# Terascale-All-sensing-Research-Studio/MOV-SLAM

Hardware: AMD Instinct MI355X
Metric: local-BA iterations/sec (50 KF x 20k MapPoint window) (higher is better)
Workload: dtype f64; 1 GPU; LocalBundleAdjustment 50 KF + 10 fixed x 20000 MapPoints, E=110510 mono edges, Huber on, 10 LM iterations (cfg3, seed 1003); one window per GPU; parallelism=1 window

## Files before the change

mov-slam_amd/csrc/kernels.h:

```cpp
#pragma once
#include <hip/hip_runtime.h>

#include "device_types.h"

namespace movba {

constexpr int kBandThreads = 512;
constexpr int kPcgRowsThreads = 512;
constexpr int kPcgPlanWaves = kPcgRowsThreads / 64, kPcgPlanOwnBatch = 10;

hipError_t configure_kernels(int unused);
hipError_t configure_pcg_rows();
hipError_t configure_struct_kernels();
hipError_t launch_struct_count(const StructDev &sd, hipStream_t s);
hipError_t launch_struct_scan(const StructDev &sd, hipStream_t s);
hipError_t launch_struct_counts_out(const StructDev &sd, int32_t *host_cnt_dev, int seq, hipStream_t s, const int32_t *basic_pe = nullptr, const int32_t *basic_info = nullptr);
hipError_t launch_ingest(const IngestArgs &a, hipStream_t s);
int ingest_workgroups();
hipError_t launch_basic(const BasicDev &bd, hipStream_t s);
bool struct_lds_fits(int nfree, int NP);
hipError_t launch_struct_fill(const StructDev &sd, hipStream_t s);
hipError_t launch_couple_count(const StructDev &sd, int32_t *cnt_pt, hipStream_t s);
size_t sorted_fill_temp_bytes(int P, long long noff, int nfree);
hipError_t launch_sorted_fill(const StructDev &sd, const int32_t *cnt_pt, int32_t *off, unsigned *keys_in, unsigned *keys_out,
                              unsigned long long *vals_in, void *tmp, size_t tmp_bytes, long long noff, hipStream_t s);
hipError_t launch_slot_point(int32_t *slot, const int32_t *g_pose, const int32_t *base, const int32_t *g_point, int32_t *slot_point, int E, const int32_t *hx, int NP, hipStream_t s);
bool pcg_rows_supported(int nfree, const int32_t *row_ptr, PcgParams *pp);
hipError_t launch_pcg_rows(const DevWindow &w, int nrowent, const PcgParams &pp, int trial, hipStream_t s);

hipError_t launch_init(const DevWindow &w, hipStream_t s);
hipError_t launch_linearize(const DevWindow &w, hipStream_t s);
hipError_t launch_schur(const DevWindow &w, int mode, hipStream_t s);
hipError_t launch_lambda_init(const DevWindow &w, hipStream_t s);
hipError_t launch_backsub(const DevWindow &w, hipStream_t s);
hipError_t launch_finalize(const DevWindow &w, hipStream_t s);
struct ExportDst { unsigned long long *poses, *points, *chi2, *outlier; };
hipError_t launch_export(const DevWindow &w, const ExportDst &d, hipStream_t s);

hipError_t launch_init_batch(const BatchDev &b, int nblk, hipStream_t s);
hipError_t launch_point_batch(const BatchDev &b, int nblk, bool backsub, bool stereo, bool ldsp, size_t lds, hipStream_t s);
size_t point_lds_bytes_for(const DevWindow &w, bool backsub, bool ldsp);
int schur_blocks(const DevWindow &w);
hipError_t launch_schur_batch(const BatchDev &b, int nblk, int mode, bool stereo, hipStream_t s);
hipError_t launch_lambda_init_batch(const BatchDev &b, hipStream_t s);
hipError_t launch_finalize_batch(const BatchDev &b, int nblk, hipStream_t s);
hipError_t launch_pcg_rows_batch(const BatchDev &b, bool overflow, bool padded, size_t lds, int trial, hipStream_t s);
size_t pcg_rows_lds_bytes(int nfree, int nrowent, bool padded);
size_t band_lds_bytes(int nfree, int bw);
bool band_supported(int nfree, int bw);
hipError_t launch_band(const DevWindow &w, int bw, hipStream_t s);
hipError_t launch_band_batch(const BatchDev &b, size_t lds, hipStream_t s);
hipError_t configure_band();

hipError_t configure_dense_kernels();
hipError_t launch_dense_solve(const DevWindow &w, hipStream_t s);
hipError_t launch_dense_factor(const DevWindow &w, hipStream_t s);
hipError_t configure_dense_persist();
bool dense_persist_supported(const DensePlan &p);
hipError_t launch_dense_persist(const DevWindow &w, unsigned epoch, hipStream_t s);
size_t dense_tiles_doubles(int nfree);
int dense_ntile(int nfree);
constexpr size_t kPointLdsLimit = 150 * 1024;
size_t point_lds_need(int NP, int nfree);

}
```

mov-slam_amd/csrc/pcg_plan.cpp:

```cpp
#include "kernels.h"

namespace movba {

namespace {
constexpr int kNW = kPcgPlanWaves, kNC = kCoarseDim, kOwnBatch = kPcgPlanOwnBatch;
}

size_t pcg_rows_lds_bytes(int nfree, int nrowent, bool padded)
{
    const size_t n = 6 * (size_t)nfree, npad = (n + 1) & ~(size_t)1;
    const size_t ypart = padded ? n * kOwnBatch + 5 * kOwnBatch + 6 + kOwnBatch : 6 * ((size_t)nrowent / 2 + 1 + kOwnBatch);
    const size_t solve = (2 * npad + 36 * (size_t)nfree + 2 * kNW + 2 + kNC * kNC / 2 + kNC + 32 * kNW + ypart + 36 * (size_t)nfree + 64 * kNW) * sizeof(double);
    const size_t coarse = ((size_t)kNC * kNC + 9 * kNC + 8) * sizeof(double) + 2 * sizeof(int32_t) * ((size_t)nrowent + 2);
    return solve > coarse ? solve : coarse;
}

size_t band_lds_bytes(int nfree, int bw)
{
    const size_t n = 6 * (size_t)nfree, npad = (n + 1) & ~(size_t)1;
    const size_t ntri = ((size_t)bw * (bw + 1) / 2 + 1) & ~(size_t)1;
    return ((size_t)nfree * (bw + 1) * 36 + 2 * npad + (size_t)bw * 36 + 8 + 12) * sizeof(double) + (ntri + 4) * sizeof(int32_t);
}

bool band_supported(int nfree, int bw) { return nfree >= 1 && bw >= 0 && bw <= 77 && band_lds_bytes(nfree, bw) <= 159 * 1024; }

bool pcg_rows_supported(int nfree, const int32_t *row_ptr, PcgParams *pp)
{
    if (nfree <= 0 || nfree > 10 * kNW) return false;
    const int nrowent = row_ptr[nfree];
    int maxrow = 0;
    for (int b = 0; b < nfree; ++b) maxrow = row_ptr[b + 1] - row_ptr[b] > maxrow ? row_ptr[b + 1] - row_ptr[b] : maxrow;
    pp->padded = 0;
    if (pcg_rows_lds_bytes(nfree, nrowent, false) > 159 * 1024) return false;
    const bool pad_fits = maxrow <= 2 * kOwnBatch && pcg_rows_lds_bytes(nfree, nrowent, true) <= 159 * 1024;
    auto fill = [&](int cap, int32_t *out) {
        int b = 0, wv = 0;
        for (; wv < kNW && b < nfree; ++wv) {
            int e = b + 1;
            while (e < nfree && e - b < 10 && row_ptr[e + 1] - row_ptr[b] <= cap) ++e;
            if (out) out[wv + 1] = e;
            b = e;
        }
        if (out) for (; wv < kNW; ++wv) out[wv + 1] = nfree;
        return b == nfree;
    };
    if (nfree <= kNW) {
        for (int wv = 0; wv <= kNW; ++wv) pp->wave_row0[wv] = wv < nfree ? wv : nfree;
        pp->overflow = 0;
        pp->padded = pad_fits ? 1 : 0;
        return true;
    }
    int lo = 1, hi = nrowent > 1 ? nrowent : 1;
    while (lo < hi) {
        const int mid = (lo + hi) / 2;
        if (fill(mid, nullptr)) hi = mid; else lo = mid + 1;
    }
    pp->wave_row0[0] = 0;
    if (!fill(lo, pp->wave_row0)) return false;
    pp->overflow = 0;
    for (int wv = 0; wv < kNW; ++wv)
        if (row_ptr[pp->wave_row0[wv + 1]] - row_ptr[pp->wave_row0[wv]] > 128) pp->overflow = 1;
    pp->padded = (pad_fits && !pp->overflow) ? 1 : 0;
    return true;
}

}
```

mov-slam_amd/csrc/structure.cpp:

```cpp
#include "structure.h"

#include <algorithm>
#include <cstdlib>
#include <cstring>

namespace movba {

void reset_structure(Structure& s, int NP, int P, int E)
{
    s.nfree = 0; s.npairs = 0; s.nitems = 0; s.max_degree = 0; s.nentries = 0; s.already_grouped = true; s.n_fixed = 0; s.n_agg = 0; s.reordered = false;
    s.free_pose.clear(); s.pair_i.clear(); s.pair_j.clear(); s.items.clear(); s.sched.clear(); s.sched_per_xcd = 0; s.row_ent.clear();
    s.cblk_g.clear(); s.cblk_h.clear(); s.cblk_ptr.clear(); s.cblk_ent.clear(); s.ent_i.clear(); s.ent_j.clear(); s.ent_l.clear(); s.E_free = 0;
    s.NP = NP; s.P = P; s.E = E;
}

void index_poses(const uint8_t* pose_fixed, Structure& s)
{
    const int NP = s.NP;
    s.hidx.assign(NP, -1);
    std::vector<int32_t>& pstart = s.pose_slot0;
    pstart.assign(NP + 1, -1);
    int run = 0;
    for (int i = 0; i < NP; ++i) {
        if (pose_fixed[i]) { s.n_fixed++; continue; }
        if (s.pose_edges[i] > 0) { s.hidx[i] = s.nfree++; s.free_pose.push_back(i); pstart[i] = run; run += s.pose_edges[i]; }
    }
    s.E_free = run;
}

int build_basic(const movba_lba_desc& d, Structure& s, int32_t* rank_out)
{
    const int NP = d.n_poses, P = d.n_points, E = d.n_edges;
    if (NP < 0 || P < 0 || E < 0) return MOVBA_ERR_ARG;
    if ((NP && (!d.poses || !d.pose_fixed)) || (P && !d.points)) return MOVBA_ERR_ARG;
    if (E && (!d.edge_pose || !d.edge_point || !d.obs || !d.inv_sigma2)) return MOVBA_ERR_ARG;
    reset_structure(s, NP, P, E);

    s.pose_edges.assign(NP + 1, 0);
    s.pt_start.assign(P + 2, 0);
    {
        bool grouped = true;
        int prev_l = -1;
        int32_t *pe = s.pose_edges.data(), *pend = s.pt_start.data() + 1;
        const int32_t *ep = d.edge_pose, *el = d.edge_point;
        for (int e = 0; e < E; ++e) {
            const int ip = ep[e], l = el[e];
            if ((unsigned)ip >= (unsigned)NP || (unsigned)l >= (unsigned)P) return MOVBA_ERR_ARG;
            const int r = pe[ip]++;
            if (rank_out) rank_out[e] = r;
            pend[l] = e + 1;
            grouped &= l >= prev_l;
            prev_l = l;
        }
        s.already_grouped = grouped;
    }
    if (s.already_grouped) {
        for (int l = 0; l < P; ++l) {
            const int b = s.pt_start[l], en = std::max(s.pt_start[l + 1], b);
            s.pt_start[l + 1] = en;
            s.max_degree = std::max(s.max_degree, en - b);
        }
        s.pt_start.pop_back();
    } else {
        std::fill(s.pt_start.begin(), s.pt_start.end(), 0);
        for (int e = 0; e < E; ++e) s.pt_start[d.edge_point[e] + 2]++;
        for (int l = 0; l < P; ++l) { s.max_degree = std::max(s.max_degree, s.pt_start[l + 2]); s.pt_start[l + 2] += s.pt_start[l + 1]; }
    }
    if (s.already_grouped) {
        s.perm.clear();
        s.gp = d.edge_pose; s.gl = d.edge_point;
    } else {
        s.perm.resize(E);
        s.g_pose.resize(E); s.g_point.resize(E);
        for (int e = 0; e < E; ++e) {
            const int pos = s.pt_start[d.edge_point[e] + 1]++;
            s.perm[pos] = e;
        }
        s.pt_start.pop_back();
        for (int g = 0; g < E; ++g) {
            s.g_pose[g] = d.edge_pose[s.perm[g]];
            s.g_point[g] = d.edge_point[s.perm[g]];
        }
        s.gp = s.g_pose.data(); s.gl = s.g_point.data();
    }
    index_poses(d.pose_fixed, s);
    if (!rank_out) build_slots(s);
    if (E == 0) return MOVBA_EMPTY;
    return MOVBA_OK;
}

void build_slots(Structure& s)
{
    s.slot.resize(s.E);
    const int32_t *gp = s.gp;
    int32_t *sl = s.slot.data(), *ps = s.pose_slot0.data();
    for (int g = 0; g < s.E; ++g) { const int i = gp[g]; const int v = ps[i]; sl[g] = v; ps[i] = v + (v >= 0); }
}

static int free_lists(const Structure& s, std::vector<int32_t>& fe_start, std::vector<int32_t>& fe_h, std::vector<int32_t>& fe_g)
{
    const int P = s.P;
    fe_start.assign(P + 1, 0); fe_h.clear(); fe_g.clear();
    fe_h.reserve(s.E); fe_g.reserve(s.E);
    for (int l = 0; l < P; ++l) {
        const size_t base = fe_h.size();
        for (int g = s.pt_start[l]; g < s.pt_start[l + 1]; ++g) {
            const int h = s.hidx[s.gp[g]];
            if (h < 0) continue;
            size_t pos = fe_h.size();
            fe_h.push_back(h); fe_g.push_back(g);
            while (pos > base && fe_h[pos - 1] > h) {
                fe_h[pos] = fe_h[pos - 1]; fe_g[pos] = fe_g[pos - 1];
                --pos;
            }
            fe_h[pos] = h; fe_g[pos] = g;
            if (pos > base && fe_h[pos - 1] == h) return MOVBA_ERR_ARG;
            if (pos + 1 < fe_h.size() && fe_h[pos + 1] == h) return MOVBA_ERR_ARG;
        }
        fe_start[l + 1] = (int32_t)fe_h.size();
    }
    return MOVBA_OK;
}

int finish_pairs(Structure& s, const int32_t* cnt)
{
    const int nf = s.nfree;
    s.pid.assign((size_t)nf * (size_t)nf, -1);
    s.pair_i.clear(); s.pair_j.clear();
    for (int i = 0; i < nf; ++i) { s.pid[(size_t)i * nf + i] = i; s.pair_i.push_back(i); s.pair_j.push_back(i); }
    for (int i = 0; i < nf; ++i)
        for (int j = i + 1; j < nf; ++j)
            if (cnt[(size_t)i * nf + j] > 0) {
                s.pid[(size_t)i * nf + j] = (int32_t)s.pair_i.size();
                s.pair_i.push_back(i); s.pair_j.push_back(j);
            }
    s.npairs = (int)s.pair_i.size();
    s.pair_ptr.assign(s.npairs + 1, 0);
    for (int p = 0; p < s.npairs; ++p) s.pair_ptr[p + 1] = s.pair_ptr[p] + cnt[(size_t)s.pair_i[p] * nf + s.pair_j[p]];
    s.nentries = s.pair_ptr[s.npairs];
    if (s.nentries > (int64_t)0x7fffffff) return MOVBA_ERR_ARG;
    if (nf > 0 && s.pair_ptr[nf] != (int64_t)s.E_free) return MOVBA_ERR_ARG;

    s.items.clear();
    s.pair_item_start.assign(s.npairs + 1, 0);
    for (int p = 0; p < s.npairs; ++p) {
        const int64_t cap = p < nf ? kSchurChunkDiag : kSchurChunk, len = s.pair_ptr[p + 1] - s.pair_ptr[p];
        const int64_t parts = (len + cap - 1) / cap;
        const int64_t chunk = parts > 0 ? ((len + parts - 1) / parts + 3) / 4 * 4 : cap;
        s.pair_item_start[p] = (int32_t)s.items.size();
        for (int64_t b = s.pair_ptr[p]; b < s.pair_ptr[p + 1]; b += chunk)
            s.items.push_back(Item{ p, (int32_t)b, (int32_t)std::min<int64_t>(b + chunk, s.pair_ptr[p + 1]), p < nf ? 1 : 0 });
    }
    s.pair_item_start[s.npairs] = (int32_t)s.items.size();
    s.nitems = (int)s.items.size();

    {
        const int ipw = kSchurWaves / kSchurWPI;
        std::vector<int32_t>& order = s.tmp_order;
        order.resize(s.nitems);
        {
            int n = 0, od = nf < s.npairs ? s.pair_item_start[nf] : s.nitems;
            for (int i = 0; i < nf; ++i) {
                for (int k = s.pair_item_start[i]; k < s.pair_item_start[i + 1]; ++k) order[n++] = k;
                while (od < s.nitems && s.pair_i[s.items[od].pair] == i) order[n++] = od++;
            }
        }
        auto weight = [&](int k) { const Item& it = s.items[k]; return (int64_t)(it.end - it.begin) * (it.diag ? 3 : 2) + 128; };
        int64_t total = 0;
        for (int k = 0; k < s.nitems; ++k) total += weight(k);
        std::vector<uint64_t>& key = s.tmp_key;
        key.resize(s.nitems);
        int seg_begin[9];
        {
            int64_t acc = 0; int x = 0;
            seg_begin[0] = 0;
            for (int n = 0; n < s.nitems; ++n) {
                while (x < 7 && acc >= (total * (x + 1)) / 8) seg_begin[++x] = n;
                const int64_t wgt = weight(order[n]);
                key[n] = ((uint64_t)(0x7fffffff - wgt) << 32) | (uint32_t)n;
                acc += wgt;
            }
            while (x < 8) seg_begin[++x] = s.nitems;
        }
#ifndef MOVBA_SCHUR_T1
#define MOVBA_SCHUR_T1 128
#define MOVBA_SCHUR_T2 256
#endif
#ifndef MOVBA_SCHUR_DW
#define MOVBA_SCHUR_DW 4
#endif
        auto waves_of = [&](int k) { const Item& it = s.items[k]; const int n = it.end - it.begin; return it.diag ? MOVBA_SCHUR_DW : (n > MOVBA_SCHUR_T2 ? 4 : (n > MOVBA_SCHUR_T1 ? 2 : 1)); };
        size_t longest = 1;
        for (int g = 0; g < 8; ++g) {
            std::sort(key.begin() + seg_begin[g], key.begin() + seg_begin[g + 1]);
            size_t slots = 0;
            for (int n = seg_begin[g]; n < seg_begin[g + 1]; ++n) {
                const size_t nw = (size_t)waves_of(order[(uint32_t)key[n]]);
                if ((slots & 3) + nw > 4) slots = (slots + 3) & ~(size_t)3;
                slots += nw;
            }
            longest = std::max(longest, (slots + 3) & ~(size_t)3);
        }
        (void)ipw;
        s.sched_per_xcd = (int)longest;
        s.sched.assign((size_t)8 * s.sched_per_xcd, SchedItem{ 0, 0, -1, 0, 0, -1, -1, 0 });
        for (int g = 0; g < 8; ++g) {
            size_t slots = 0;
            for (int n = seg_begin[g]; n < seg_begin[g + 1]; ++n) {
                const int item = order[(uint32_t)key[n]];
                const Item& it = s.items[item];
                const int nw = waves_of(item);
                if ((slots & 3) + (size_t)nw > 4) slots = (slots + 3) & ~(size_t)3;
                const int len = it.end - it.begin, epw = (len + nw - 1) / nw;
                for (int sub = 0; sub < nw; ++sub) {
                    const int wb = std::min(it.begin + sub * epw, it.end), we = std::min(wb + epw, it.end);
                    s.sched[(size_t)g * s.sched_per_xcd + slots + sub] = SchedItem{ wb, we, (item << 1) | (it.diag ? 1 : 0),
                                                                                   s.free_pose[s.pair_i[it.pair]], s.free_pose[s.pair_j[it.pair]], -1, -1, sub | (nw << 8) };
                }
                slots += (size_t)nw;
            }
        }
    }

    {
        s.row_ptr.assign(nf + 1, 0);
        for (int p = 0; p < s.npairs; ++p) {
            s.row_ptr[s.pair_i[p] + 1]++;
            if (p >= nf) s.row_ptr[s.pair_j[p] + 1]++;
        }
        for (int i = 0; i < nf; ++i) s.row_ptr[i + 1] = s.row_ptr[i] + ((s.row_ptr[i + 1] + 1) & ~1);
        s.row_ent.assign((size_t)s.row_ptr[nf], RowEnt{ -1, 0, 0, 0 });
        std::vector<int32_t>& cur = s.tmp_order;
        cur.assign(s.row_ptr.begin(), s.row_ptr.begin() + nf);
        for (int p = nf; p < s.npairs; ++p) s.row_ent[cur[s.pair_j[p]]++] = RowEnt{ p, s.pair_i[p], 1, 0 };
        for (int i = 0; i < nf; ++i) s.row_ent[cur[i]++] = RowEnt{ i, i, 0, 0 };
        for (int p = nf; p < s.npairs; ++p) s.row_ent[cur[s.pair_i[p]]++] = RowEnt{ p, s.pair_j[p], 0, 0 };
    }
    return MOVBA_OK;
}

bool covisibility_order(int nf, const int32_t* cnt, std::vector<int32_t>& new_of_old)
{
    new_of_old.resize(nf);
    for (int i = 0; i < nf; ++i) new_of_old[i] = i;
    if (nf < 3) return false;
    auto linked = [&](int a, int b) { return a == b ? false : (a < b ? cnt[(size_t)a * nf + b] : cnt[(size_t)b * nf + a]) > 0; };
    std::vector<int32_t> deg(nf, 0);
    for (int i = 0; i < nf; ++i) for (int j = i + 1; j < nf; ++j) if (cnt[(size_t)i * nf + j] > 0) { deg[i]++; deg[j]++; }
    auto envelope = [&](const std::vector<int32_t>& old_of_new) {
        int64_t env = 0;
        for (int r = 0; r < nf; ++r) {
            int first = r;
            for (int c = 0; c < r; ++c) if (linked(old_of_new[r], old_of_new[c])) { first = c; break; }
            env += r - first;
        }
        return env;
    };
    std::vector<int32_t> order, level(nf), queue;
    std::vector<uint8_t> placed(nf, 0);
    auto bfs = [&](int root, std::vector<int32_t>& out) {
        out.clear(); out.push_back(root);
        std::fill(level.begin(), level.end(), -1); level[root] = 0;
        for (size_t h = 0; h < out.size(); ++h) {
            const int v = out[h];
            const size_t first = out.size();
            for (int u = 0; u < nf; ++u) if (!placed[u] && level[u] < 0 && linked(v, u)) { level[u] = level[v] + 1; out.push_back(u); }
            std::sort(out.begin() + first, out.end(), [&](int a, int b) { return deg[a] != deg[b] ? deg[a] < deg[b] : a < b; });
        }
        return level[out.back()];
    };
    order.reserve(nf);
    for (;;) {
        int root = -1;
        for (int i = 0; i < nf; ++i) if (!placed[i] && (root < 0 || deg[i] < deg[root])) root = i;
        if (root < 0) break;
        for (int sweep = 0; sweep < 2; ++sweep) {
            const int depth = bfs(root, queue);
            int far = -1;
            for (int v : queue) if (level[v] == depth && (far < 0 || deg[v] < deg[far])) far = v;
            if (far == root) break;
            root = far;
        }
        bfs(root, queue);
        for (int v : queue) { placed[v] = 1; order.push_back(v); }
    }
    std::reverse(order.begin(), order.end());
    std::vector<int32_t> natural(nf);
    for (int i = 0; i < nf; ++i) natural[i] = i;
    const int64_t env_nat = envelope(natural), env_rcm = envelope(order);
    if (!(env_rcm * 5 < env_nat * 4)) return false;
    for (int k = 0; k < nf; ++k) new_of_old[order[k]] = k;
    return true;
}

void apply_pose_order(Structure& s, const std::vector<int32_t>& new_of_old, int32_t* cnt)
{
    const int nf = s.nfree;
    std::vector<int32_t> fp(nf);
    for (int h = 0; h < nf; ++h) fp[new_of_old[h]] = s.free_pose[h];
    s.free_pose = fp;
    for (int h = 0; h < nf; ++h) s.hidx[s.free_pose[h]] = h;
    int run = 0;
    for (int h = 0; h < nf; ++h) { s.pose_slot0[s.free_pose[h]] = run; run += s.pose_edges[s.free_pose[h]]; }
    if (cnt) {
        std::vector<int32_t> c2((size_t)nf * nf, 0);
        for (int i = 0; i < nf; ++i)
            for (int j = i; j < nf; ++j) {
                const int a = new_of_old[i], b = new_of_old[j];
                c2[(size_t)std::min(a, b) * nf + std::max(a, b)] = cnt[(size_t)i * nf + j];
            }
        std::memcpy(cnt, c2.data(), sizeof(int32_t) * c2.size());
    }
}

int build_structure(const movba_lba_desc& d, Structure& s)
{
    const int rc = build_basic(d, s);
    if (rc != MOVBA_OK) return rc;
    const int P = s.P, nf = s.nfree;

    std::vector<int32_t> fe_start, fe_h, fe_g;
    const int rf = free_lists(s, fe_start, fe_h, fe_g);
    if (rf != MOVBA_OK) return rf;
    std::vector<int32_t> cnt((size_t)nf * (size_t)nf, 0);
    for (int l = 0; l < P; ++l)
        for (int a = fe_start[l]; a < fe_start[l + 1]; ++a) {
            int32_t *row = &cnt[(size_t)fe_h[a] * nf];
            for (int b = a; b < fe_start[l + 1]; ++b) row[fe_h[b]]++;
        }
    if (nf <= 80 && !s.no_reorder) {
        std::vector<int32_t> new_of_old;
        if (covisibility_order(nf, cnt.data(), new_of_old)) {
            apply_pose_order(s, new_of_old, nullptr);
            build_slots(s);
            const int rf2 = free_lists(s, fe_start, fe_h, fe_g);
            if (rf2 != MOVBA_OK) return rf2;
            std::fill(cnt.begin(), cnt.end(), 0);
            for (int l = 0; l < P; ++l)
                for (int a = fe_start[l]; a < fe_start[l + 1]; ++a) {
                    int32_t *row = &cnt[(size_t)fe_h[a] * nf];
                    for (int b = a; b < fe_start[l + 1]; ++b) row[fe_h[b]]++;
                }
            s.reordered = true;
        }
    }
    const int rp = finish_pairs(s, cnt.data());
    if (rp != MOVBA_OK) return rp;
    if (s.pair_ptr[nf] != s.E_free) return MOVBA_ERR_ARG;
    const size_t noff = (size_t)(s.nentries - s.E_free);
    s.ent_i.resize(noff); s.ent_j.resize(noff); s.ent_l.resize(noff);
    {
        std::vector<int32_t> cur(s.npairs);
        for (int p = 0; p < s.npairs; ++p) cur[p] = (int32_t)(s.pair_ptr[p] - s.E_free);
        for (int l = 0; l < P; ++l)
            for (int a = fe_start[l]; a < fe_start[l + 1]; ++a) {
                const int32_t *prow = &s.pid[(size_t)fe_h[a] * nf];
                const int32_t ga = fe_g[a];
                for (int b = a + 1; b < fe_start[l + 1]; ++b) {
                    const int32_t pos = cur[prow[fe_h[b]]]++;
                    s.ent_i[pos] = s.slot[ga]; s.ent_j[pos] = s.slot[fe_g[b]]; s.ent_l[pos] = l;
                }
            }
    }
    return MOVBA_OK;
}

void build_coarse(Structure& s, const int32_t* agg_row0, int n_agg)
{
    const int nf = s.nfree, G = n_agg;
    s.n_agg = G;
    s.cblk_g.clear(); s.cblk_h.clear(); s.cblk_ent.clear(); s.cblk_ij.clear(); s.cblk_ptr.assign(1, 0);
    s.multi_pairs.clear();
    for (int p = nf; p < s.npairs; ++p)
        if (s.pair_item_start[p + 1] - s.pair_item_start[p] > 1) s.multi_pairs.push_back(p);
    std::vector<int32_t> agg_of(nf, 0);
    for (int g = 0; g < G; ++g)
        for (int i = agg_row0[g]; i < agg_row0[g + 1]; ++i) agg_of[i] = g;
    std::vector<std::vector<int32_t>> lists((size_t)G * G), ijs((size_t)G * G);
    for (int i = 0; i < nf; ++i)
        for (int e = s.row_ptr[i]; e < s.row_ptr[i + 1]; ++e)
            if (s.row_ent[e].block >= 0) {
                const size_t b = (size_t)agg_of[i] * G + agg_of[s.row_ent[e].col];
                const int pr = s.row_ent[e].block;
                const bool single = pr >= nf && s.pair_item_start[pr + 1] - s.pair_item_start[pr] == 1;
                const int src_idx = single ? s.pair_item_start[pr] : pr;
                lists[b].push_back((src_idx << 2) | (s.row_ent[e].transposed ? 2 : 0) | (single ? 1 : 0));
                ijs[b].push_back((i << 16) | s.row_ent[e].col);
            }
    for (int g = 0; g < G; ++g)
        for (int h = 0; h < G; ++h) {
            const std::vector<int32_t>& l = lists[(size_t)g * G + h];
            if (l.empty()) continue;
            s.cblk_g.push_back(g); s.cblk_h.push_back(h);
            s.cblk_ent.insert(s.cblk_ent.end(), l.begin(), l.end());
            s.cblk_ij.insert(s.cblk_ij.end(), ijs[(size_t)g * G + h].begin(), ijs[(size_t)g * G + h].end());
            s.cblk_ptr.push_back((int32_t)s.cblk_ent.size());
        }
}

}
```

mov-slam_amd/csrc/structure.h:

```cpp
#pragma once
#include <cstdint>
#include <vector>

#include "movba.h"

namespace movba {

struct Int2 { int32_t x, y; };
struct Int4 { int32_t x, y, z, w; };
struct Item { int32_t pair, begin, end, diag; };
struct SchedItem {
    int32_t begin, end, tag , pose_i, pose_j ;
    int32_t dst_a, dst_b;
    int32_t sub;
};
struct RowEnt { int32_t block, col, transposed, pad; };

struct Structure {
    int NP = 0, P = 0, E = 0, nfree = 0;
    int npairs = 0, nitems = 0, max_degree = 0;
    int64_t nentries = 0;
    bool already_grouped = true;
    bool reordered = false;
    bool no_reorder = false;
    int n_fixed = 0;
    std::vector<int32_t> hidx;
    std::vector<int32_t> free_pose;
    std::vector<int32_t> perm;
    std::vector<int32_t> tmp_order; std::vector<uint64_t> tmp_key;
    std::vector<int32_t> pose_edges, pose_slot0;
    std::vector<int32_t> pt_start;
    std::vector<int32_t> g_pose, g_point;
    const int32_t *gp = nullptr, *gl = nullptr;
    std::vector<int32_t> pair_i, pair_j;
    std::vector<int32_t> pair_item_start;
    std::vector<int64_t> pair_ptr;
    std::vector<int32_t> pid;
    std::vector<int32_t> slot;
    std::vector<int32_t> ent_i, ent_j, ent_l;
    int E_free = 0;
    std::vector<Item> items;
    std::vector<SchedItem> sched;
    int sched_per_xcd = 0;
    std::vector<int32_t> row_ptr;
    std::vector<RowEnt> row_ent;
    int n_agg = 0;
    std::vector<int32_t> cblk_g, cblk_h, cblk_ptr;
    std::vector<int32_t> cblk_ent;
    std::vector<int32_t> multi_pairs;
    std::vector<int32_t> cblk_ij;
};

void build_coarse(Structure& s, const int32_t* agg_row0, int n_agg);

#ifndef MOVBA_SCHUR_WAVES
#define MOVBA_SCHUR_WAVES 4
#define MOVBA_SCHUR_WPI 4
#define MOVBA_SCHUR_EPW 512
#endif
#ifndef MOVBA_SCHUR_EPW_DIAG
#define MOVBA_SCHUR_EPW_DIAG 128
#endif
constexpr int kSchurWaves = MOVBA_SCHUR_WAVES;
constexpr int kSchurWPI = MOVBA_SCHUR_WPI;
constexpr int kSchurChunkDiag = MOVBA_SCHUR_EPW_DIAG * kSchurWPI;
constexpr int kSchurChunk = MOVBA_SCHUR_EPW * kSchurWPI;

int build_structure(const movba_lba_desc& d, Structure& s);
int build_basic(const movba_lba_desc& d, Structure& s, int32_t* rank_out = nullptr);
void reset_structure(Structure& s, int NP, int P, int E);
void index_poses(const uint8_t* pose_fixed, Structure& s);
void build_slots(Structure& s);
int finish_pairs(Structure& s, const int32_t* cnt);

bool covisibility_order(int nf, const int32_t* cnt, std::vector<int32_t>& new_of_old);
void apply_pose_order(Structure& s, const std::vector<int32_t>& new_of_old, int32_t* cnt );

}
```

mov-slam_amd/csrc/upload.cpp:

```cpp
#include <algorithm>
#include <cmath>
#include <cstring>
#include <vector>

#include "handle.h"
#include "kernels.h"

using namespace movba;

namespace {

inline void put(void *dst, const void *src, size_t bytes) { if (bytes) std::memcpy(dst, src, bytes); }

struct EdgeLayout {
    size_t gpose = 0, ptstart = 0, hidx = 0;
    size_t a_end = 0;
    size_t gpoint = 0, free_pose = 0, slot = 0;
    size_t base = 0;
    size_t raw_begin = 0, obs = 0, isig = 0, obsr = 0, pose0 = 0, point0 = 0, kcam = 0;
    size_t grouped_end = 0;
    size_t perm = 0;
    size_t max_end = 0;
    bool has_kcam = false;
};

constexpr int kSortedMaxPoses = 1024;

constexpr int kDeviceStructureMinEdges = 2048;

struct HelperHandOff {
    std::atomic<int> idx_ready{0};

    hipError_t copy_err = hipSuccess;
    hipError_t idx_err = hipSuccess;
    char *arena = nullptr;
    uint64_t arena_gen = 0;
    bool joined = false;
};

void pack_kcam(double *kc, const movba_lba_desc *d, int np)
{
    for (int i = 0; i < np; ++i) {
        const double *ck = d->cam_kf ? d->cam_kf + 4 * (size_t)i : &d->fx;
        kc[8 * i] = ck[0]; kc[8 * i + 1] = ck[1]; kc[8 * i + 2] = ck[2]; kc[8 * i + 3] = ck[3];
        kc[8 * i + 4] = d->bf_kf ? d->bf_kf[i] : d->bf; kc[8 * i + 5] = kc[8 * i + 6] = kc[8 * i + 7] = 0.0;
    }
}

struct SlotPointLaunch {
    int32_t *slot;
    const int32_t *g_pose, *base, *g_point;
    int32_t *slot_point;
    int E;
    const int32_t *hx;
    int NP;
};
hipError_t queue_slot_point(const SlotPointLaunch &a, hipStream_t s)
{
    return launch_slot_point(a.slot, a.g_pose, a.base, a.g_point, a.slot_point, a.E, a.hx, a.NP, s);
}

struct FillLaunch {
    StructDev sd{};
    bool scan_first = false;
    const int32_t *cnt_pt = nullptr;
    int32_t *off = nullptr;
    unsigned *keys_in = nullptr, *keys_out = nullptr;
    unsigned long long *vals_in = nullptr;
    void *tmp = nullptr;
    size_t tmp_bytes = 0;
    long long noff = 0;
};
hipError_t queue_fill(const FillLaunch &f, hipStream_t s)
{
    if (f.scan_first) { const hipError_t e = launch_struct_scan(f.sd, s); if (e != hipSuccess) return e; }
    if (f.cnt_pt) return launch_sorted_fill(f.sd, f.cnt_pt, f.off, f.keys_in, f.keys_out, f.vals_in, f.tmp, f.tmp_bytes, f.noff, s);
    return launch_struct_fill(f.sd, s);
}

struct EarlySetup {
    SlotPointLaunch slots;
    FillLaunch fill;
    DevWindow win;
    int delay_us;
    bool laps;
    double t0;
};

struct Upload {
    movba_handle *const h;
    const movba_lba_desc *const d;
    const int NP, P, E;
    Carver c;
    EdgeLayout L;
    HelperHandOff ho;
    char *sg = nullptr;
    size_t misc_bytes = 0;
    bool stereo = false;
    bool done = false;
    bool rank_mode = true;
    int nf = 0, nb = 0, nbins = 0;
    size_t edge_bytes = 0;
    uint64_t arena_gen_at_edge_copy = 0;
    bool edge_b_early = false, edge_b_stale = false, edge_b_queued = false;
    double upload_host_ms = 0.0;
    int nf_expect = 0;
    bool raw_synced = false;
    bool direct_raw = false;
    bool dev_first = false;
    BasicDev bd{};
    size_t so_cnt = 0, so_err = 0, so_ent0 = 0, so_cntw = 0, so_cntpt = 0, so_pe = 0, so_info = 0, so_fixed = 0, so_H = 0;
    volatile int32_t *misc_seq = nullptr;
    int32_t seq = 0;
    StructDev sd{};
    bool dev_structure = false, ent_packed = false, filled_early = false;
    bool scan_pending = false;
    bool sorted_structure = false;
    size_t s2_off = 0, s2_keys_in = 0, s2_keys_out = 0, s2_vals_in = 0, s2_tmp = 0, s2_tmp_bytes = 0;
    uint64_t fill_gen = 0;
    size_t noff = 0, o_ent = 0, o_slotpt = 0;
    size_t pair_begin = 0, hole = 0, h2d = 0, total = 0;
    size_t o_items = 0, o_sched = 0, o_pi = 0, o_pj = 0, o_pis = 0, o_rowptr = 0, o_rowent = 0, o_plan = 0;
    size_t o_cg = 0, o_ch = 0, o_cp = 0, o_ce = 0, o_cij = 0, o_multi = 0, o_pid = 0, o_prange = 0, o_dtp = 0, o_dtk = 0;
    size_t o_st[2][11] = {};
    size_t o_obspm = 0, o_obsrpm = 0, o_part = 0, o_blocks = 0, o_blocks_ov = 0, o_blocks_c = 0, o_aci = 0, o_acitag = 0;
    size_t o_bp = 0, o_xp = 0, o_scale = 0, o_hmax = 0, o_tick = 0, o_recd = 0, o_imgb = 0, o_ctrl = 0, o_chi2 = 0, o_outl = 0;
    size_t o_dtiles = 0, o_ddiag = 0, o_dfail = 0, o_dx = 0, o_dflags = 0, o_dcontrib = 0, o_dstamps = 0;
    std::vector<int32_t> lane_plan;
    int rec_slots = 1;
    size_t ncb = 0;
    int ntile = 0;
    bool dense_one = false, dense_stamps = false;
    double t0 = 0.0, lap_t = 0.0;
    bool lap_on = false;

    Upload(movba_handle *h_, const movba_lba_desc *d_) : h(h_), d(d_), NP(d_->n_poses), P(d_->n_points), E(d_->n_edges) {}
    ~Upload() { h->packer.wait(); if (direct_raw && !raw_synced) (void)hipStreamSynchronize(h->copy_stream); }

    const Structure &s() const { return h->st; }
    void lap(const char *what)
    {
        if (!lap_on) return;
        const double t = now_ms();
        std::fprintf(stderr, "libmovba[upload]: %-28s %.3f ms\n", what, t - lap_t);
        lap_t = t;
    }
    int join_helper()
    {
        if (ho.joined) return MOVBA_OK;
        h->packer.wait();
        ho.joined = true;
        if (ho.copy_err != hipSuccess) { std::fprintf(stderr, "libmovba: upload copy failed: %s\n", hipGetErrorString(ho.copy_err)); return MOVBA_ERR_HIP; }
        return MOVBA_OK;
    }

    int run(bool allow_dev_first);
    int begin();
    void post_helper();
    int group();
    bool dev_first_eligible() const;
    int group_on_device();
    void carve_state();
    bool state_carved = false;
    int pack_derived();
    int send_edge_a();
    int structure_on_host();
    int structure_on_device();
    int structure_on_device_sorted();
    void choose_solver();
    int lay_out_rest();
    void pack_pairs();
    int send_pairs();
    void device_view();
    void pack_a(bool raw_too);
    void pack_b(bool raw_too);
    void pack_edges(bool raw_too) { pack_a(raw_too); pack_b(raw_too); }
    int queue_edge_b();
    int carve_scratch(bool basic);
    void start_struct_dev();
    void aim_struct_dev();
    int launch_counts();
    int counts_out(const int32_t *basic_pe, const int32_t *basic_info);
    int wait_for_counts();
    int after_counts();
    int carve_entries();
    int finish_structure();
    SlotPointLaunch slot_point_launch() const;
    FillLaunch next_fill();
    int queue_slots_and_fill();
    int post_early_setup();
    DevWindow state_view() const;
    size_t ent_words() const { return (ent_packed ? 2 : 3) * noff + 4; }
    char *sp(size_t o) const { return sg + (o - hole); }
    int32_t *misc() const { return reinterpret_cast<int32_t *>(sg + h->stage_cap - misc_bytes); }
};

int Upload::begin()
{
    HIP_TRY(hipSetDevice(h->device));
    h->uploaded = false; h->ran = false; h->early_status = MOVBA_OK; h->early_setup = false;
    t0 = lap_t = now_ms();
    lap_on = process_switches().time_upload;
    if (NP < 0 || P < 0 || E < 0) return MOVBA_ERR_ARG;
    if ((NP && (!d->poses || !d->pose_fixed)) || (P && !d->points)) return MOVBA_ERR_ARG;
    if (E && (!d->edge_pose || !d->edge_point || !d->obs || !d->inv_sigma2)) return MOVBA_ERR_ARG;
    L.gpose = c.take<int32_t>(E); L.ptstart = c.take<int32_t>(P + 1); L.hidx = c.take<int32_t>(NP);
    L.a_end = c.off;
    L.gpoint = c.take<int32_t>(E);
    L.free_pose = c.take<int32_t>(NP + 1);
    L.slot = c.take<int32_t>(E);
    L.base = c.take<int32_t>(NP + 1);
    L.raw_begin = c.off;
    L.obs = c.take<double>(2 * (size_t)E); L.isig = c.take<double>(E);
    L.obsr = c.take<double>(d->obs_right ? E : 0);
    L.pose0 = c.take<double>(7 * (size_t)NP); L.point0 = c.take<double>(3 * (size_t)P);
    L.has_kcam = d->cam_kf || d->bf_kf;
    L.kcam = c.take<double>(L.has_kcam ? 8 * (size_t)NP : 0);
    L.grouped_end = c.off;
    L.perm = c.take<int32_t>(E);
    L.max_end = c.off;
    const size_t nf_dev = (size_t)(NP <= kSortedMaxPoses ? NP : 80);
    misc_bytes = (nf_dev * nf_dev + 8) * sizeof(int32_t) * 2 + 4096 + sizeof(int32_t) * ((size_t)std::min(NP, 1024) + kBasicInfo + 8);
    int rc = ensure_stage(h, L.max_end + misc_bytes); if (rc) return rc;
    if (L.max_end > h->arena_cap) { rc = ensure_arena(h, 10 * L.max_end); if (rc) return rc; }
    HIP_TRY(hipStreamSynchronize(h->stream));
    HIP_TRY(hipStreamSynchronize(h->copy_stream));
    sg = h->stage;
    if (d->obs_right) for (int e = 0; e < E && !stereo; ++e) stereo = d->obs_right[e] >= 0.0;
    return MOVBA_OK;
}

void Upload::post_helper()
{
    ho.arena = h->arena;
    ho.arena_gen = h->arena_gen;
    const EdgeLayout lay = L;
    char *const stage = sg;
    movba_handle *const hh = h;
    const movba_lba_desc *const dd = d;
    const int np = NP, p = P, e = E;
    HelperHandOff *const out = &ho;
    if (direct_raw) {
        h->packer.post([=]() {
            hipError_t err = hipSetDevice(hh->device);
            auto dma = [&](size_t to, const void *from, size_t bytes) {
                if (err == hipSuccess && bytes) err = hipMemcpyAsync(out->arena + to, from, bytes, hipMemcpyHostToDevice, hh->copy_stream);
            };
            dma(lay.obs, dd->obs, sizeof(double) * 2 * (size_t)e);
            dma(lay.isig, dd->inv_sigma2, sizeof(double) * (size_t)e);
            if (dd->obs_right) dma(lay.obsr, dd->obs_right, sizeof(double) * (size_t)e);
            dma(lay.point0, dd->points, sizeof(double) * 3 * (size_t)p);
            dma(lay.pose0, dd->poses, sizeof(double) * 7 * (size_t)np);
            if (lay.has_kcam) {
                pack_kcam(reinterpret_cast<double *>(stage + lay.kcam), dd, np);
                dma(lay.kcam, stage + lay.kcam, sizeof(double) * 8 * (size_t)np);
            }
            if (err == hipSuccess) err = hipEventRecord(hh->copy_event, hh->copy_stream);
            out->copy_err = err;
        });
        ho.idx_ready.store(1, std::memory_order_release);
        return;
    }
    const int helper_delay_us = HOOK(h, helper_delay_us);
    const bool send_idx = dev_first;
    h->packer.post([=]() {
        if (helper_delay_us > 0) std::this_thread::sleep_for(std::chrono::microseconds(helper_delay_us));
        std::memcpy(stage + lay.gpose, dd->edge_pose, sizeof(int32_t) * (size_t)e);
        std::memcpy(stage + lay.gpoint, dd->edge_point, sizeof(int32_t) * (size_t)e);
        if (send_idx) {
            hipError_t e0 = hipSetDevice(hh->device);
            if (e0 == hipSuccess) e0 = hipMemcpyAsync(out->arena + lay.gpose, stage + lay.gpose, sizeof(int32_t) * (size_t)e, hipMemcpyHostToDevice, hh->copy_stream);
            if (e0 == hipSuccess) e0 = hipMemcpyAsync(out->arena + lay.gpoint, stage + lay.gpoint, sizeof(int32_t) * (size_t)e, hipMemcpyHostToDevice, hh->copy_stream);
            if (e0 == hipSuccess) e0 = hipEventRecord(hh->edgeb_event, hh->copy_stream);
            out->idx_err = e0;
        }
        out->idx_ready.store(1, std::memory_order_release);
        hipError_t err = hipSetDevice(hh->device);
        auto send = [&](size_t from, size_t to) {
            if (err == hipSuccess && to > from)
                err = hipMemcpyAsync(out->arena + from, stage + from, to - from, hipMemcpyHostToDevice, hh->copy_stream);
        };
        std::memcpy(stage + lay.obs, dd->obs, sizeof(double) * 2 * (size_t)e);
        send(lay.obs, lay.isig);
        std::memcpy(stage + lay.isig, dd->inv_sigma2, sizeof(double) * (size_t)e);
        if (dd->obs_right) std::memcpy(stage + lay.obsr, dd->obs_right, sizeof(double) * (size_t)e);
        std::memcpy(stage + lay.pose0, dd->poses, sizeof(double) * 7 * (size_t)np);
        std::memcpy(stage + lay.point0, dd->points, sizeof(double) * 3 * (size_t)p);
        if (lay.has_kcam) pack_kcam(reinterpret_cast<double *>(stage + lay.kcam), dd, np);
        send(lay.isig, lay.grouped_end);
        if (err == hipSuccess) err = hipEventRecord(hh->copy_event, hh->copy_stream);
        out->copy_err = err;
    });
}

int Upload::group()
{
    h->st.no_reorder = h->opt.reorder == -1;
    const int rc = build_basic(*d, h->st, reinterpret_cast<int32_t *>(sg + L.slot));
    rank_mode = true;
    lap("build_basic");
    if (rc < 0) { (void)join_helper(); (void)hipStreamSynchronize(h->copy_stream); return rc; }
    h->stop = d->stop;
    if (rc == MOVBA_EMPTY || s().P == 0) { h->early_status = MOVBA_EMPTY; }
    else if (s().n_fixed == 0) { h->early_status = MOVBA_NO_FIXED; }
    if (h->early_status != MOVBA_OK) {
        const int rw = join_helper(); if (rw) return rw;
        h->prof.structure_ms += now_ms() - t0; h->uploaded = true; done = true; return MOVBA_OK;
    }
    nf = s().nfree;
    if (nf > MOVBA_MAX_FREE_KEYFRAMES) {
        (void)join_helper();
        std::fprintf(stderr, "libmovba: %d free keyframes: the reduced system exceeds the direct solver's capacity (%d)\n", nf, MOVBA_MAX_FREE_KEYFRAMES);
        return MOVBA_ERR_TOO_LARGE;
    }
    nb = (P + kPointsPerBlock - 1) / kPointsPerBlock;
    edge_bytes = s().already_grouped ? L.grouped_end : L.max_end;
    nbins = nf * nf;
    return MOVBA_OK;
}

void Upload::carve_state()
{
    for (int b = 0; b < 2; ++b) {
        o_st[b][0] = c.take<double>(7 * (size_t)NP); o_st[b][1] = c.take<double>(12 * (size_t)NP);
        o_st[b][2] = c.take<double>(3 * (size_t)P);  o_st[b][3] = c.take<double>(6 * (size_t)P);
        o_st[b][4] = c.take<double>(3 * (size_t)P);  o_st[b][5] = c.take<double>(4 * (size_t)E);
        o_st[b][6] = 0;  o_st[b][7] = 0;
        o_st[b][8] = c.take<double>(nb);
        o_st[b][9] = 0;
        o_st[b][10] = 0;
    }
    o_obspm = c.take<double>(2 * (size_t)E + 2); o_obsrpm = c.take<double>(stereo ? (size_t)E + 1 : 1);
    o_aci = c.take<double>(3 * kCoarseDim * kCoarseDim + 2); o_acitag = c.take<int32_t>(2);
    o_bp = c.take<double>(6 * (size_t)nf + 1); o_xp = c.take<double>(6 * (size_t)nf + 1);
    o_scale = c.take<double>(nb + 1); o_hmax = c.take<double>(nb); o_tick = c.take<uint32_t>(8 * (size_t)nb + 8);
    o_ctrl = c.take<Ctrl>(1); o_chi2 = c.take<double>(E); o_outl = c.take<uint8_t>(E);
    state_carved = true;
}

bool Upload::dev_first_eligible() const
{
    if (HOOK(h, host_structure) || HOOK(h, host_grouping)) return false;
    if (E < kDeviceStructureMinEdges) return false;
    if (E <= 0 || P <= 0 || NP <= 0 || NP > 1024) return false;
    int nfix = 0;
    for (int i = 0; i < NP; ++i) nfix += d->pose_fixed[i] != 0;
    const int nfm = NP - nfix;
    return nfix > 0 && nfm > 0 && nfm <= 80 && struct_lds_fits(nfm, NP);
}

constexpr int kRetryClassic = 1 << 20;
int Upload::group_on_device()
{
    Structure &st = h->st;
    reset_structure(st, NP, P, E);
    st.no_reorder = h->opt.reorder == -1;
    for (nf_expect = 0, nf = 0; nf < NP; ++nf) nf_expect += d->pose_fixed[nf] == 0;
    nf = nf_expect; nbins = nf * nf;
    nb = (P + kPointsPerBlock - 1) / kPointsPerBlock;
    edge_bytes = L.grouped_end;
    carve_state();
    int rc = carve_scratch(true); if (rc) return rc;
    char *sa = h->scratch.p;
    std::memcpy(sg + L.hidx, d->pose_fixed, (size_t)NP);
    const size_t zero_bytes = so_info + sizeof(int32_t) * kBasicInfo - so_cnt;
    if (!direct_raw) HIP_TRY(hipMemsetAsync(sa + so_cnt, 0, zero_bytes, h->stream));
    bd = BasicDev{};
    bd.E = E; bd.P = P; bd.NP = NP; bd.nblk = (E + kBasicBlock - 1) / kBasicBlock;
    if (direct_raw) {
        auto view = [](const void *p, size_t bytes) { return static_cast<const void *>(host_block_view(p, bytes)); };
        IngestArgs ia{};
        ia.seg[0] = IngestSeg{ view(d->edge_pose, sizeof(int32_t) * (size_t)E), h->arena + L.gpose, sizeof(int32_t) * (size_t)E };
        ia.seg[1] = IngestSeg{ view(d->edge_point, sizeof(int32_t) * (size_t)E), h->arena + L.gpoint, sizeof(int32_t) * (size_t)E };
        ia.seg[2] = IngestSeg{ h->stage_dev + L.hidx, sa + so_fixed, ((size_t)NP + 3) & ~(size_t)3 };
        ia.nseg = 3; ia.counter = h->ingest_counter; ia.wait_for = 0;
        ia.zero = reinterpret_cast<unsigned *>(sa + so_cnt); ia.zero_words = (unsigned)(zero_bytes / 4);
        HIP_TRY(launch_ingest(ia, h->stream));
        h->ingest_expect += (unsigned)ingest_workgroups();

    } else {
        while (ho.idx_ready.load(std::memory_order_acquire) == 0) host_relax(h->opt.host_wait);
        if (ho.idx_err != hipSuccess) { std::fprintf(stderr, "libmovba: upload copy failed: %s\n", hipGetErrorString(ho.idx_err)); return MOVBA_ERR_HIP; }
        HIP_TRY(hipStreamWaitEvent(h->stream, h->edgeb_event, 0));
    }
    arena_gen_at_edge_copy = ho.arena_gen;
    bd.edge_pose = reinterpret_cast<const int32_t *>(h->arena + L.gpose); bd.edge_point = reinterpret_cast<const int32_t *>(h->arena + L.gpoint);
    bd.pose_fixed = direct_raw ? reinterpret_cast<const uint8_t *>(sa + so_fixed) : reinterpret_cast<const uint8_t *>(h->stage_dev + L.hidx);
    bd.pt_start = reinterpret_cast<int32_t *>(h->arena + L.ptstart); bd.rank = reinterpret_cast<int32_t *>(h->arena + L.slot);
    bd.H = reinterpret_cast<int32_t *>(sa + so_H); bd.pose_edges = reinterpret_cast<int32_t *>(sa + so_pe);
    bd.hidx = reinterpret_cast<int32_t *>(h->arena + L.hidx); bd.base = reinterpret_cast<int32_t *>(h->arena + L.base);
    bd.free_pose = reinterpret_cast<int32_t *>(h->arena + L.free_pose); bd.info = reinterpret_cast<int32_t *>(sa + so_info);
    HIP_TRY(launch_basic(bd, h->stream));
    rc = launch_counts(); if (rc) return rc;
    lap("grouping + count launches");
    rc = wait_for_counts(); if (rc) return rc;
    const int32_t *info = misc() + nbins + 2, *pe = info + kBasicInfo;
    if (info[0]) { (void)join_helper(); (void)hipStreamSynchronize(h->copy_stream); return MOVBA_ERR_ARG; }
    if (info[1] || info[2] != nf_expect) return kRetryClassic;
    st.pose_edges.assign(pe, pe + NP); st.pose_edges.push_back(0);
    index_poses(d->pose_fixed, st);
    if (st.nfree != nf_expect || st.E_free != info[3]) return MOVBA_ERR_HIP;
    st.already_grouped = true; st.perm.clear(); st.gp = d->edge_pose; st.gl = d->edge_point;
    st.pt_start.clear();
    rank_mode = true;
    h->stop = d->stop;
    lap("wait for the grouping pass and the pair counts");
    return MOVBA_OK;
}

void Upload::pack_a(bool raw_too)
{
    if (!s().already_grouped || raw_too) {
        put(sg + L.gpose, s().gp, sizeof(int32_t) * E);
        put(sg + L.gpoint, s().gl, sizeof(int32_t) * E);
    }
    put(sg + L.ptstart, s().pt_start.data(), sizeof(int32_t) * (P + 1));
    put(sg + L.hidx, s().hidx.data(), sizeof(int32_t) * NP);
}

void Upload::pack_b(bool raw_too)
{
    if (!s().already_grouped) put(sg + L.perm, s().perm.data(), sizeof(int32_t) * E);
    if (!rank_mode) put(sg + L.slot, s().slot.data(), sizeof(int32_t) * E);
    else put(sg + L.base, s().pose_slot0.data(), sizeof(int32_t) * NP);
    put(sg + L.free_pose, s().free_pose.data(), sizeof(int32_t) * nf);
    double *obs = reinterpret_cast<double *>(sg + L.obs), *isg = reinterpret_cast<double *>(sg + L.isig);
    double *obr = reinterpret_cast<double *>(sg + L.obsr);
    if (!s().already_grouped) {
        for (int g = 0; g < E; ++g) {
            const int e = s().perm[g];
            obs[2 * g] = d->obs[2 * e]; obs[2 * g + 1] = d->obs[2 * e + 1]; isg[g] = d->inv_sigma2[e];
        }
        if (d->obs_right) for (int g = 0; g < E; ++g) obr[g] = d->obs_right[s().perm[g]];
    } else if (raw_too) {
        put(obs, d->obs, sizeof(double) * 2 * (size_t)E);
        put(isg, d->inv_sigma2, sizeof(double) * (size_t)E);
        if (d->obs_right) put(obr, d->obs_right, sizeof(double) * (size_t)E);
    }
    if (raw_too) {
        put(sg + L.pose0, d->poses, sizeof(double) * 7 * (size_t)NP);
        put(sg + L.point0, d->points, sizeof(double) * 3 * (size_t)P);
    }
}

int Upload::pack_derived()
{
    if (!s().already_grouped) {
        const int rw = join_helper(); if (rw) return rw;
        HIP_TRY(hipEventSynchronize(h->copy_event));
        build_slots(h->st); rank_mode = false;
        pack_edges(false);
    } else {
        while (ho.idx_ready.load(std::memory_order_acquire) == 0) host_relax(h->opt.host_wait);
        pack_a(false);
        pack_b(false);
    }
    lap("pack derived arrays");
    return MOVBA_OK;
}

int Upload::send_edge_a()
{
    const double t_up0 = now_ms();
    HIP_TRY(hipMemcpyAsync(h->arena, sg, L.a_end, hipMemcpyHostToDevice, h->stream));
    arena_gen_at_edge_copy = ho.arena_gen;
    if (s().already_grouped && h->arena_gen == ho.arena_gen && E >= kDeviceStructureMinEdges && !HOOK(h, host_structure)) {
        HIP_TRY(hipMemcpyAsync(h->arena + L.a_end, sg + L.a_end, L.raw_begin - L.a_end, hipMemcpyHostToDevice, h->copy_stream));
        HIP_TRY(hipEventRecord(h->edgeb_event, h->copy_stream));
        edge_b_early = true;
    }
    upload_host_ms = now_ms() - t_up0;
    return MOVBA_OK;
}

int Upload::queue_edge_b()
{
    if (dev_first) { edge_b_queued = true; return MOVBA_OK; }
    if (edge_b_early) HIP_TRY(hipStreamWaitEvent(h->stream, h->edgeb_event, 0));
    if (!edge_b_early || edge_b_stale) {
        HIP_TRY(hipMemcpyAsync(h->arena + L.a_end, sg + L.a_end, L.raw_begin - L.a_end, hipMemcpyHostToDevice, h->stream));
    }
    if (!s().already_grouped) {
        { const int rw = join_helper(); if (rw) return rw; }
        HIP_TRY(hipStreamWaitEvent(h->stream, h->copy_event, 0));
        HIP_TRY(hipMemcpyAsync(h->arena + L.raw_begin, sg + L.raw_begin, edge_bytes - L.raw_begin, hipMemcpyHostToDevice, h->stream));
    }
    edge_b_queued = true;
    return MOVBA_OK;
}

int Upload::structure_on_host()
{
    const int rc = build_structure(*d, h->st);
    if (rc < 0) return rc;
    rank_mode = false;
    pack_b(false); edge_b_stale = true;
    noff = (size_t)(s().nentries - s().E_free);
    o_slotpt = c.take<int32_t>((size_t)s().E_free + 1);
    return MOVBA_OK;
}

int Upload::carve_scratch(bool basic)
{
    const int nchunks = (P + 63) / 64;
    Carver sc;
    so_cnt = sc.take<int32_t>(nbins); so_err = sc.take<int32_t>(4);
    so_pe = sc.take<int32_t>(basic ? NP : 0); so_info = sc.take<int32_t>(basic ? kBasicInfo : 0);
    so_ent0 = sc.take<int32_t>(nbins);
    so_cntw = sc.take<int32_t>(sorted_structure ? 0 : (size_t)nbins * nchunks);
    so_cntpt = sc.take<int32_t>(sorted_structure ? (size_t)P + 1 : 0);
    so_fixed = sc.take<uint8_t>(basic ? (size_t)NP + 4 : 0);
    so_H = sc.take<int32_t>(basic ? (size_t)((E + kBasicBlock - 1) / kBasicBlock) * NP : 0);
    return h->scratch.grow(h, sc.off);
}

void Upload::start_struct_dev()
{
    char *sa = h->scratch.p;
    sd = StructDev{};
    sd.P = P; sd.nfree = nf; sd.NP = NP;
    if (!sorted_structure) { sd.nchunks = (P + 63) / 64; sd.cntw = reinterpret_cast<int32_t *>(sa + so_cntw); }
    sd.cnt = reinterpret_cast<int32_t *>(sa + so_cnt); sd.error = reinterpret_cast<int32_t *>(sa + so_err);
    sd.ent0 = reinterpret_cast<int32_t *>(sa + so_ent0);
    sd.abort = dev_first ? reinterpret_cast<const int32_t *>(sa + so_info) : nullptr;
    aim_struct_dev();
}

void Upload::aim_struct_dev()
{
    char *a = h->arena;
    sd.g_pose = reinterpret_cast<int32_t *>(a + L.gpose); sd.pt_start = reinterpret_cast<int32_t *>(a + L.ptstart);
    sd.hidx = reinterpret_cast<int32_t *>(a + L.hidx);
    sd.slot = reinterpret_cast<const int32_t *>(a + L.slot);
    if (!o_ent) return;
    int32_t *ed = reinterpret_cast<int32_t *>(a + o_ent);
    sd.ent_i = ed; sd.ent_j = ed + noff; sd.ent_l = ed + 2 * noff;
    sd.ent64 = ent_packed ? reinterpret_cast<unsigned long long *>(a + o_ent) : nullptr;
}

int Upload::launch_counts()
{
    start_struct_dev();
    HIP_TRY(launch_struct_count(sd, h->stream));
    const int rc = counts_out(dev_first ? reinterpret_cast<const int32_t *>(h->scratch.p + so_pe) : nullptr,
                              dev_first ? reinterpret_cast<const int32_t *>(h->scratch.p + so_info) : nullptr);
    if (rc) return rc;
    scan_pending = dev_first && direct_raw && h->opt.profile == 0;
    if (!scan_pending) HIP_TRY(launch_struct_scan(sd, h->stream));
    return MOVBA_OK;
}

int Upload::counts_out(const int32_t *basic_pe, const int32_t *basic_info)
{
    misc_seq = reinterpret_cast<volatile int32_t *>(misc()) + nbins + 1;
    seq = (int32_t)(++h->count_seq & 0x7fffffff);
    __atomic_store_n(misc_seq, seq - 1, __ATOMIC_RELAXED);
    HIP_TRY(launch_struct_counts_out(sd, reinterpret_cast<int32_t *>(h->stage_dev + h->stage_cap - misc_bytes), seq, h->stream, basic_pe, basic_info));
    return MOVBA_OK;
}

int Upload::wait_for_counts()
{
    const double t_wait = now_ms();
    while (__atomic_load_n(misc_seq, __ATOMIC_ACQUIRE) != seq) {
        host_relax(h->opt.host_wait);
        if (now_ms() - t_wait > 10000.0) { HIP_TRY(hipStreamSynchronize(h->stream)); if (__atomic_load_n(misc_seq, __ATOMIC_ACQUIRE) != seq) return MOVBA_ERR_HIP; }
    }
    return MOVBA_OK;
}

int Upload::structure_on_device()
{
    int rc = carve_scratch(false); if (rc) return rc;
    HIP_TRY(hipMemsetAsync(h->scratch.p + so_cnt, 0, so_err + 16 - so_cnt, h->stream));
    rc = launch_counts(); if (rc) return rc;
    lap("edge H2D + count launches");
    return after_counts();
}

int Upload::after_counts()
{
    int32_t *cnt = misc();
    if (!dev_first) { const int rc = wait_for_counts(); if (rc) return rc; }
    if (cnt[nbins] != 0) return MOVBA_ERR_ARG;
    lap("wait for the pair counts");
    if (!h->st.no_reorder) {
        std::vector<int32_t> new_of_old;
        if (covisibility_order(nf, cnt, new_of_old)) {
            apply_pose_order(h->st, new_of_old, cnt);
            h->st.reordered = true;
            std::memcpy(sg + L.hidx, s().hidx.data(), sizeof(int32_t) * NP);
            std::memcpy(sg + L.base, s().pose_slot0.data(), sizeof(int32_t) * NP);
            std::memcpy(sg + L.free_pose, s().free_pose.data(), sizeof(int32_t) * nf);
            HIP_TRY(hipMemcpyAsync(h->arena + L.hidx, sg + L.hidx, sizeof(int32_t) * NP, hipMemcpyHostToDevice, h->stream));
            if (dev_first) {
                HIP_TRY(hipMemcpyAsync(h->arena + L.base, sg + L.base, sizeof(int32_t) * NP, hipMemcpyHostToDevice, h->stream));
                HIP_TRY(hipMemcpyAsync(h->arena + L.free_pose, sg + L.free_pose, sizeof(int32_t) * nf, hipMemcpyHostToDevice, h->stream));
            } else edge_b_stale = true;
            HIP_TRY(hipMemsetAsync(h->scratch.p + so_cnt, 0, so_err + 16 - so_cnt, h->stream));
            HIP_TRY(launch_struct_count(sd, h->stream));
            HIP_TRY(launch_struct_counts_out(sd, nullptr, 0, h->stream));
            HIP_TRY(launch_struct_scan(sd, h->stream));
            scan_pending = false;
            lap("covisibility reorder + recount");
        }
    }
    int rc = queue_edge_b(); if (rc) return rc;
    rc = carve_entries(); if (rc) return rc;
    if (c.off <= h->arena_cap && h->arena_gen == ho.arena_gen) {
        filled_early = true; fill_gen = h->arena_gen;
        if (dev_first && direct_raw && h->opt.profile == 0) rc = post_early_setup();
        else rc = queue_slots_and_fill();
        if (rc) return rc;
    }
    lap("edge B H2D + fill kernel (queued)");
    return finish_structure();
}

int Upload::carve_entries()
{
    const int32_t *cnt = misc();
    int64_t n = 0;
    for (int i = 0; i < nf; ++i) for (int j = i + 1; j < nf; ++j) n += cnt[(size_t)i * nf + j];
    if (n > (int64_t)0x7fffffff / 4) return MOVBA_ERR_ARG;
    noff = (size_t)n;
    o_ent = c.take<int32_t>(ent_words());
    o_slotpt = c.take<int32_t>((size_t)s().E_free + 1);
    aim_struct_dev();
    return MOVBA_OK;
}

int Upload::finish_structure()
{
    const int rc = finish_pairs(h->st, misc());
    lap("finish_pairs");
    if (rc < 0) return rc;
    if ((size_t)(s().nentries - s().E_free) != noff) return MOVBA_ERR_ARG;
    return MOVBA_OK;
}

int Upload::structure_on_device_sorted()
{
    sorted_structure = true;
    int rc = carve_scratch(false); if (rc) return rc;
    HIP_TRY(hipMemsetAsync(h->scratch.p + so_cnt, 0, so_err + 16 - so_cnt, h->stream));
    start_struct_dev();
    HIP_TRY(launch_couple_count(sd, reinterpret_cast<int32_t *>(h->scratch.p + so_cntpt), h->stream));
    rc = counts_out(nullptr, nullptr); if (rc) return rc;
    lap("edge H2D + count launches");
    rc = wait_for_counts(); if (rc) return rc;
    if (misc()[nbins] != 0) return MOVBA_ERR_ARG;
    lap("wait for the pair counts");
    rc = queue_edge_b(); if (rc) return rc;
    rc = carve_entries(); if (rc) return rc;
    Carver s2;
    s2_off = s2.take<int32_t>((size_t)P + 1);
    s2_keys_in = s2.take<unsigned>(noff + 1); s2_keys_out = s2.take<unsigned>(noff + 1);
    s2_vals_in = s2.take<unsigned long long>(noff + 1);
    s2_tmp_bytes = sorted_fill_temp_bytes(P, (long long)noff, nf);
    s2_tmp = s2.take<char>(s2_tmp_bytes);
    rc = h->scratch2.grow(h, s2.off); if (rc) return rc;
    if (c.off <= h->arena_cap && h->arena_gen == ho.arena_gen) {
        rc = queue_slots_and_fill(); if (rc) return rc;
        filled_early = true; fill_gen = h->arena_gen;
    }
    lap("edge B H2D + fill kernels (queued)");
    return finish_structure();
}

SlotPointLaunch Upload::slot_point_launch() const
{
    char *a = h->arena;
    return SlotPointLaunch{ reinterpret_cast<int32_t *>(a + L.slot), reinterpret_cast<const int32_t *>(a + L.gpose),
                            rank_mode ? reinterpret_cast<const int32_t *>(a + L.base) : nullptr, reinterpret_cast<const int32_t *>(a + L.gpoint),
                            reinterpret_cast<int32_t *>(a + o_slotpt), E, dev_first ? reinterpret_cast<const int32_t *>(h->scratch.p + so_H) : nullptr, NP };
}

FillLaunch Upload::next_fill()
{
    FillLaunch f;
    f.sd = sd;
    f.scan_first = scan_pending;
    scan_pending = false;
    if (sorted_structure) {
        char *s2 = h->scratch2.p;
        f.cnt_pt = reinterpret_cast<const int32_t *>(h->scratch.p + so_cntpt); f.off = reinterpret_cast<int32_t *>(s2 + s2_off);
        f.keys_in = reinterpret_cast<unsigned *>(s2 + s2_keys_in); f.keys_out = reinterpret_cast<unsigned *>(s2 + s2_keys_out);
        f.vals_in = reinterpret_cast<unsigned long long *>(s2 + s2_vals_in);
        f.tmp = s2 + s2_tmp; f.tmp_bytes = s2_tmp_bytes; f.noff = (long long)noff;
    }
    return f;
}

int Upload::queue_slots_and_fill()
{
    HIP_TRY(queue_slot_point(slot_point_launch(), h->stream));
    if (dev_structure) HIP_TRY(queue_fill(next_fill(), h->stream));
    return MOVBA_OK;
}

int Upload::post_early_setup()
{
    { const int rw = join_helper(); if (rw) return rw; }
    const EarlySetup es{ slot_point_launch(), next_fill(), state_view(), HOOK(h, helper_delay_us), lap_on, t0 };
    const int device = h->device;
    const hipStream_t stream = h->stream;
    const hipEvent_t copy_event = h->copy_event;
    HelperHandOff *const out = &ho;
    h->packer.post([es, device, stream, copy_event, out]() {
        if (es.delay_us > 0) std::this_thread::sleep_for(std::chrono::microseconds(es.delay_us));
        double tl[6]; tl[0] = now_ms();
        hipError_t err = hipSetDevice(device);
        if (err == hipSuccess) err = queue_slot_point(es.slots, stream);
        tl[1] = now_ms();
        if (err == hipSuccess) err = queue_fill(es.fill, stream);
        tl[2] = now_ms();
        if (err == hipSuccess) err = hipStreamWaitEvent(stream, copy_event, 0);
        tl[3] = now_ms();
        if (err == hipSuccess) err = launch_init(es.win, stream);
        tl[4] = now_ms();
        if (err == hipSuccess) err = launch_linearize(es.win, stream);
        tl[5] = now_ms();
        out->copy_err = err;
        if (es.laps) std::fprintf(stderr, "libmovba[upload]: helper's launches (ms into the call): start %.3f, slots %.3f, scan + fill %.3f, event wait %.3f, init %.3f, linearise %.3f\n",
                                  tl[0] - es.t0, tl[1] - es.t0, tl[2] - es.t0, tl[3] - es.t0, tl[4] - es.t0, tl[5] - es.t0);
    });
    ho.joined = false;
    h->early_setup = true;
    return MOVBA_OK;
}

void Upload::choose_solver()
{
    h->pp = PcgParams{};
    h->rows_kernel = pcg_rows_supported(s().nfree, s().row_ptr.data(), &h->pp);
    if (HOOK(h, pcg_packed)) h->pp.padded = 0;
    {
        const bool over = h->rows_kernel && h->pp.overflow;
        if (h->rows_kernel && ((over && !h->opt.pcg_spill) || h->opt.solver == 1)) h->rows_kernel = false;
    }
    {
        int bw = 0;
        for (int p = nf; p < s().npairs; ++p) bw = std::max(bw, (int)(s().pair_j[p] - s().pair_i[p]));
        h->band_bw = bw;
        const int band_env = process_switches().band;
        double m_sum = 0.0;
        for (int k = 0; k < nf; ++k) m_sum += std::min(bw, nf - 1 - k);
        const double m_avg = nf > 0 ? m_sum / nf : 0.0;
        const double rt = std::ceil((m_avg * (m_avg + 1.0) * 18.0 + 6.0 * m_avg) / 512.0), rp = std::max(1.0, std::ceil(m_avg * 36.0 / 512.0));
        const double est = nf * (1970.0 + 780.0 * rp + 420.0 * rt) + 54.0 * nf * (bw + 1) + 360.0 * nf + 5000.0;
        const bool forced = h->opt.solver == 2 || (h->opt.solver == 0 && band_env == 1);
        const bool off = h->opt.solver == 3 || h->opt.solver == 1 || (h->opt.solver == 0 && band_env == 0);
        const bool want = forced || (h->rows_kernel && est <= 130000.0);
        h->band = want && !off && band_supported(nf, bw);
    }
    if (h->rows_kernel && !h->band) build_coarse(h->st, h->pp.wave_row0, kPcgRowsThreads / 64);
    lap("pcg plan + coarse lists");
}

int Upload::lay_out_rest()
{
    pair_begin = c.off; hole = pair_begin - L.max_end;
    o_items = c.take<Item>((size_t)s().nitems + 1); o_sched = c.take<SchedItem>(s().sched.size() + 1);
    o_pi = c.take<int32_t>(s().npairs + 1); o_pj = c.take<int32_t>(s().npairs + 1); o_pis = c.take<int32_t>(s().npairs + 1);
    o_rowptr = c.take<int32_t>(nf + 1); o_rowent = c.take<RowEnt>(s().row_ent.size() + 1);
    lane_plan.clear();
    if (h->rows_kernel) {
        lane_plan.assign((size_t)kPcgRowsThreads * 12, -1);
        for (int wv = 0; wv < kPcgRowsThreads / 64; ++wv) {
            const int r0 = h->pp.wave_row0[wv], r1 = h->pp.wave_row0[wv + 1];
            const int P0 = s().row_ptr[r0] >> 1, P1 = s().row_ptr[r1] >> 1;
            for (int ln = 0; ln < 64 && P0 + ln < P1; ++ln)
                for (int k = 0; k < 2; ++k) {
                    const RowEnt &re = s().row_ent[2 * (P0 + ln) + k];
                    int32_t *pl = &lane_plan[((size_t)(wv * 64 + ln) * 3 + k) * 4];
                    if (re.block < 0) continue;
                    pl[0] = re.block; pl[1] = (re.col * 6) | (re.transposed ? (1 << 30) : 0);
                    pl[2] = s().pair_item_start[re.block]; pl[3] = s().pair_item_start[re.block + 1];
                }
            for (int ln = 0; ln < 64; ++ln) {
                int32_t *pl = &lane_plan[((size_t)(wv * 64 + ln) * 3 + 2) * 4];
                pl[0] = pl[1] = pl[2] = pl[3] = 0;
                if (ln >= 6 * (r1 - r0)) continue;
                const int bi = r0 + ln / 6;
                pl[0] = s().pair_item_start[bi]; pl[1] = s().pair_item_start[bi + 1]; pl[2] = s().row_ptr[bi]; pl[3] = s().row_ptr[bi + 1];
            }
        }
        for (int wv = 0; wv <= kPcgRowsThreads / 64; ++wv) h->pp.wave_ent0[wv] = s().row_ptr[h->pp.wave_row0[wv]];
        h->pp.nrowent = s().row_ptr[nf];
    }
    rec_slots = 1;
    for (int hh = 0; hh < nf; ++hh) rec_slots = std::max(rec_slots, (int)(s().pair_item_start[hh + 1] - s().pair_item_start[hh]));
    for (SchedItem &si : h->st.sched) {
        si.dst_a = -1; si.dst_b = -1;
        if (si.tag >= 0 && (si.tag & 1)) { const Item &it = s().items[(size_t)(si.tag >> 1)]; si.dst_a = it.pair * rec_slots + ((si.tag >> 1) - s().pair_item_start[it.pair]); }
    }
    if (h->rows_kernel && !h->pp.overflow) {
        std::vector<int32_t> slot_of_item((size_t)s().nitems, -1);
        for (size_t q = 0; q < s().sched.size(); ++q)
            if (s().sched[q].tag >= 0 && (s().sched[q].sub & 0xff) == 0) slot_of_item[(size_t)(s().sched[q].tag >> 1)] = (int32_t)q;
        for (int t = 0; t < kPcgRowsThreads; ++t)
            for (int k = 0; k < 2; ++k) {
                const int32_t *pl = &lane_plan[((size_t)t * 3 + k) * 4];
                if (pl[0] < nf || pl[3] - pl[2] != 1) continue;
                SchedItem &si = h->st.sched[(size_t)slot_of_item[(size_t)pl[2]]];
                const int32_t dst = 36 * k * kPcgRowsThreads + t;
                if ((pl[1] >> 30) & 1) si.dst_b = dst; else si.dst_a = dst;
            }
    }
    ncb = s().cblk_g.size();
    o_plan = c.take<int32_t>(lane_plan.size() + 4);
    o_cg = c.take<int32_t>(ncb + 1); o_ch = c.take<int32_t>(ncb + 1); o_cp = c.take<int32_t>(ncb + 2); o_ce = c.take<int32_t>(s().cblk_ent.size() + 1);
    o_cij = c.take<int32_t>(s().cblk_ij.size() + 1); o_multi = c.take<int32_t>(s().multi_pairs.size() + 1);
    o_pid = c.take<int32_t>((size_t)nf * nf + 1);
    ntile = dense_ntile(nf);
    const bool dense_multi = process_switches().dense_multilaunch;
    const int dense_groups = std::min(kDenseMaxGroups, h->device_cus - std::max(1, h->device_cus / 32));
    if (h->dplan_nt != ntile) { build_dense_plan(ntile, h->dplan, std::max(dense_groups, 1)); h->dplan_nt = ntile; }
    dense_one = !dense_multi && dense_groups >= 8 && dense_persist_supported(h->dplan);
    o_dtp = c.take<int32_t>(dense_one ? h->dplan.task_ptr.size() : 1); o_dtk = c.take<DenseTask>(dense_one ? h->dplan.tasks.size() : 1);
    o_prange = c.take<int32_t>(dense_one ? 2 * (size_t)nf * nf : 1);
    if (!dev_structure) o_ent = c.take<int32_t>(ent_words());
    h2d = c.off;
    if (!state_carved) carve_state();
    const size_t part_stride = ((size_t)s().nitems * kPartStride + 31) / 32 * 32;
    o_part = c.take<double>(part_stride + 1); o_blocks = c.take<double>((size_t)s().npairs * 36 + 1);
    o_recd = c.take<double>((size_t)nf * rec_slots * 48 + 2); o_imgb = c.take<double>((size_t)72 * kPcgRowsThreads);
    o_blocks_ov = c.take<double>(h->rows_kernel && h->pp.overflow ? s().row_ent.size() * 36 + 2 : 2);
    o_blocks_c = c.take<double>((size_t)s().npairs * 36 + 1);
    o_dtiles = c.take<double>(dense_tiles_doubles(nf)); o_ddiag = c.take<double>((size_t)ntile * kDenseNB * kDenseNB + 1); o_dfail = c.take<int32_t>(4);
    o_dx = c.take<double>((size_t)ntile * kDenseNB + 1);
    o_dflags = c.take<uint32_t>(dense_one ? (size_t)dense_flag_words(ntile) : 8);
    o_dcontrib = c.take<double>(dense_one ? (size_t)ntile * ntile * kDenseNB : 1);
    dense_stamps = process_switches().dense_stamps;
    o_dstamps = c.take<unsigned long long>(dense_one && dense_stamps ? 6 * h->dplan.tasks.size() : 1);
    total = c.off;

    if (total > h->arena_cap || h2d - hole + misc_bytes > h->stage_cap) { const int rw = join_helper(); if (rw) return rw; }
    int rc = ensure_arena(h, total); if (rc) return rc;
    if (dev_first && (h->arena_gen != arena_gen_at_edge_copy || h2d - hole + misc_bytes > h->stage_cap)) return kRetryClassic;
    if (h->arena_gen != arena_gen_at_edge_copy) {
        HIP_TRY(hipMemcpyAsync(h->arena, sg, edge_bytes, hipMemcpyHostToDevice, h->stream));
        aim_struct_dev();
    }
    if (h2d - hole + misc_bytes > h->stage_cap) {
        rc = ensure_stage(h, h2d - hole + misc_bytes); if (rc) return rc;
        sg = h->stage;
        pack_edges(true);
    }
    return MOVBA_OK;
}

void Upload::pack_pairs()
{
    if (!dev_structure && noff) {
        int32_t *eh = reinterpret_cast<int32_t *>(sp(o_ent));
        if (ent_packed) {
            unsigned long long *e64 = reinterpret_cast<unsigned long long *>(eh);
            for (size_t k = 0; k < noff; ++k) e64[k] = ent_pack(s().ent_i[k], s().ent_j[k], s().ent_l[k]);
        } else {
            put(eh, s().ent_i.data(), sizeof(int32_t) * noff); put(eh + noff, s().ent_j.data(), sizeof(int32_t) * noff);
            put(eh + 2 * noff, s().ent_l.data(), sizeof(int32_t) * noff);
        }
    }
    put(sp(o_items), s().items.data(), sizeof(Item) * (size_t)s().nitems);
    put(sp(o_sched), s().sched.data(), sizeof(SchedItem) * s().sched.size());
    put(sp(o_pi), s().pair_i.data(), sizeof(int32_t) * s().npairs);
    put(sp(o_pj), s().pair_j.data(), sizeof(int32_t) * s().npairs);
    put(sp(o_pis), s().pair_item_start.data(), sizeof(int32_t) * (s().npairs + 1));
    put(sp(o_rowptr), s().row_ptr.data(), sizeof(int32_t) * (nf + 1));
    put(sp(o_rowent), s().row_ent.data(), sizeof(RowEnt) * s().row_ent.size());
    if (!lane_plan.empty()) put(sp(o_plan), lane_plan.data(), sizeof(int32_t) * lane_plan.size());
    put(sp(o_cg), s().cblk_g.data(), sizeof(int32_t) * ncb);
    put(sp(o_ch), s().cblk_h.data(), sizeof(int32_t) * ncb);
    put(sp(o_cp), s().cblk_ptr.data(), sizeof(int32_t) * s().cblk_ptr.size());
    put(sp(o_ce), s().cblk_ent.data(), sizeof(int32_t) * s().cblk_ent.size());
    put(sp(o_cij), s().cblk_ij.data(), sizeof(int32_t) * s().cblk_ij.size());
    put(sp(o_multi), s().multi_pairs.data(), sizeof(int32_t) * s().multi_pairs.size());
    put(sp(o_pid), s().pid.data(), sizeof(int32_t) * (size_t)nf * nf);
    if (dense_one) {
        put(sp(o_dtp), h->dplan.task_ptr.data(), sizeof(int32_t) * h->dplan.task_ptr.size());
        put(sp(o_dtk), h->dplan.tasks.data(), sizeof(DenseTask) * h->dplan.tasks.size());
        int32_t *pr = reinterpret_cast<int32_t *>(sp(o_prange));
        for (size_t q = 0; q < (size_t)nf * nf; ++q) {
            const int32_t pair = s().pid[q];
            pr[2 * q] = pair >= 0 ? s().pair_item_start[pair] : 0;
            pr[2 * q + 1] = pair >= 0 ? s().pair_item_start[pair + 1] : 0;
        }
    }
    lap("carve + pack pair region");
}

int Upload::send_pairs()
{
    const double t2 = now_ms();
    h->prof.structure_ms += (t2 - t0) - upload_host_ms;
    if (h2d - pair_begin <= (size_t)1 << 20) {
        IngestArgs ia{};
        ia.seg[0] = IngestSeg{ h->stage_dev + L.max_end, h->arena + pair_begin, ((h2d - pair_begin) + 3) & ~(size_t)3 };
        ia.nseg = 1; ia.counter = nullptr; ia.wait_for = 0;
        HIP_TRY(launch_ingest(ia, h->stream));
    } else
        HIP_TRY(hipMemcpyAsync(h->arena + pair_begin, sg + L.max_end, h2d - pair_begin, hipMemcpyHostToDevice, h->stream));
    if (!(filled_early && fill_gen == h->arena_gen)) { const int rq = queue_slots_and_fill(); if (rq) return rq; }
    { const int rw = join_helper(); if (rw) return rw; }
    HIP_TRY(hipStreamWaitEvent(h->stream, h->copy_event, 0));
    if (direct_raw) { HIP_TRY(hipEventSynchronize(h->copy_event)); raw_synced = true; }
    lap("pair H2D (queued)");
    h->prof.upload_ms += now_ms() - t2 + upload_host_ms;
    h->h2d_bytes = h2d;
    return MOVBA_OK;
}

DevWindow Upload::state_view() const
{
    char *a = h->arena;
    DevWindow w{};
    w.NP = NP; w.P = P; w.E = E; w.nfree = nf; w.n_pt_blocks = nb;
    w.max_iters = d->max_iters; w.flags = d->flags; w.max_trials = d->max_trials > 0 ? d->max_trials : 10;
    w.fx = d->fx; w.fy = d->fy; w.cx = d->cx; w.cy = d->cy; w.huber_delta = d->huber_delta; w.chi2_gate = d->chi2_gate;
    w.g_pose = reinterpret_cast<int32_t *>(a + L.gpose); w.g_point = reinterpret_cast<int32_t *>(a + L.gpoint);
    w.pt_start = reinterpret_cast<int32_t *>(a + L.ptstart); w.perm = s().already_grouped ? nullptr : reinterpret_cast<int32_t *>(a + L.perm);
    w.hidx = reinterpret_cast<int32_t *>(a + L.hidx); w.free_pose = reinterpret_cast<int32_t *>(a + L.free_pose);
    w.obs = reinterpret_cast<double *>(a + L.obs); w.isig = reinterpret_cast<double *>(a + L.isig);
    w.obs_r = d->obs_right ? reinterpret_cast<double *>(a + L.obsr) : nullptr; w.bf = d->bf; w.stereo = stereo ? 1 : 0;
    w.kcam = L.has_kcam ? reinterpret_cast<const double *>(a + L.kcam) : nullptr;
    w.slot = reinterpret_cast<int32_t *>(a + L.slot);
    w.obs_pm = reinterpret_cast<double *>(a + o_obspm); w.obsr_pm = reinterpret_cast<double *>(a + o_obsrpm);
    {
        const int32_t *ed = reinterpret_cast<const int32_t *>(a + o_ent);
        w.ent_i = ed; w.ent_j = ed + noff; w.ent_l = ed + 2 * noff;
        w.ent64 = ent_packed ? reinterpret_cast<const unsigned long long *>(a + o_ent) : nullptr;
        w.slot_point = reinterpret_cast<const int32_t *>(a + o_slotpt); w.n_diag = s().E_free;
    }
    w.pose0 = reinterpret_cast<double *>(a + L.pose0); w.point0 = reinterpret_cast<double *>(a + L.point0);
    for (int b = 0; b < 2; ++b) {
        DevState &S = w.st[b];
        S.pose = reinterpret_cast<double *>(a + o_st[b][0]); S.Rt = reinterpret_cast<double *>(a + o_st[b][1]);
        S.point = reinterpret_cast<double *>(a + o_st[b][2]); S.Hll = reinterpret_cast<double *>(a + o_st[b][3]);
        S.bl = reinterpret_cast<double *>(a + o_st[b][4]); S.erecA = reinterpret_cast<double *>(a + o_st[b][5]);
        S.Fpart = reinterpret_cast<double *>(a + o_st[b][8]);
    }
    w.aci = reinterpret_cast<float *>(a + o_aci); w.ac_prev = reinterpret_cast<double *>(a + o_aci) + 2 * kCoarseDim * kCoarseDim; w.aci_tag = reinterpret_cast<int32_t *>(a + o_acitag);
    w.bp = reinterpret_cast<double *>(a + o_bp); w.xp = reinterpret_cast<double *>(a + o_xp);
    w.scale_part = reinterpret_cast<double *>(a + o_scale); w.hmax_part = reinterpret_cast<double *>(a + o_hmax);
    w.dec_rec = reinterpret_cast<unsigned *>(a + o_tick);
    w.ctrl = reinterpret_cast<Ctrl *>(a + o_ctrl); w.hstat = h->hstat_dev; w.ctrl_out = h->ctrl_host_dev;
    w.out_chi2 = reinterpret_cast<double *>(a + o_chi2); w.out_outlier = reinterpret_cast<uint8_t *>(a + o_outl);
    w.wait_ticks = 2000000ull;
    w.lds_poses = point_lds_need(NP, nf) <= kPointLdsLimit ? 1 : 0;
    return w;
}

void Upload::device_view()
{
    DevWindow &w = h->win;
    char *a = h->arena;
    w = state_view();
    w.npairs = s().npairs; w.nitems = s().nitems;
    w.items = reinterpret_cast<Item *>(a + o_items);
    w.sched = reinterpret_cast<SchedItem *>(a + o_sched); w.sched_per_xcd = s().sched_per_xcd;
    w.pair_i = reinterpret_cast<int32_t *>(a + o_pi); w.pair_j = reinterpret_cast<int32_t *>(a + o_pj);
    w.pair_item_start = reinterpret_cast<int32_t *>(a + o_pis); w.row_ptr = reinterpret_cast<int32_t *>(a + o_rowptr);
    w.row_ent = reinterpret_cast<RowEnt *>(a + o_rowent);
    w.lane_plan = reinterpret_cast<int32_t *>(a + o_plan);
    w.n_agg = s().n_agg; w.n_cblk = (int32_t)ncb;
    w.cblk_g = reinterpret_cast<int32_t *>(a + o_cg); w.cblk_h = reinterpret_cast<int32_t *>(a + o_ch);
    w.cblk_ptr = reinterpret_cast<int32_t *>(a + o_cp); w.cblk_ent = reinterpret_cast<int32_t *>(a + o_ce);
    w.cblk_ij = reinterpret_cast<int32_t *>(a + o_cij);
    w.multi_pairs = reinterpret_cast<int32_t *>(a + o_multi); w.n_multi = (int32_t)s().multi_pairs.size();
    w.part = reinterpret_cast<double *>(a + o_part); w.blocks = reinterpret_cast<double *>(a + o_blocks);
    w.rec_d = reinterpret_cast<double *>(a + o_recd); w.img_b = reinterpret_cast<double *>(a + o_imgb); w.rec_slots = rec_slots;
    w.blocks_c = reinterpret_cast<double *>(a + o_blocks_c); w.blocks_ov = reinterpret_cast<double *>(a + o_blocks_ov);
    w.dense.tiles = reinterpret_cast<double *>(a + o_dtiles); w.dense.diagL = reinterpret_cast<double *>(a + o_ddiag);
    w.dense.pid = reinterpret_cast<const int32_t *>(a + o_pid); w.dense.fail = reinterpret_cast<int32_t *>(a + o_dfail);
    w.dense.prange = dense_one ? reinterpret_cast<const int32_t *>(a + o_prange) : nullptr;
    w.dense.ntile = ntile; w.dense.n = 6 * nf; w.dense.xsol = reinterpret_cast<double *>(a + o_dx);
    w.dense.task_ptr = reinterpret_cast<const int32_t *>(a + o_dtp); w.dense.tasks = reinterpret_cast<const DenseTask *>(a + o_dtk);
    w.dense.flags = reinterpret_cast<unsigned *>(a + o_dflags); w.dense.failw = w.dense.flags + dense_flag_count(ntile);
    w.dense.ctag = w.dense.flags + dense_ctag_word(ntile);
    w.dense.contrib = reinterpret_cast<double *>(a + o_dcontrib);
    w.dense.stamps = dense_one && dense_stamps ? reinterpret_cast<unsigned long long *>(a + o_dstamps) : nullptr;
    w.dense.G = dense_one ? h->dplan.G : 0; w.dense.slots = dense_one ? h->dplan.slots : 0;
    h->dense_flags_clean = false; h->dense_epoch = 0;
    w.direct_only = h->rows_kernel ? 0 : 1;
}
int Upload::run(bool allow_dev_first)
{
    int rc = begin(); if (rc) return rc;
    dev_first = allow_dev_first && dev_first_eligible();
    if (dev_first) {
        direct_raw = host_block_view(d->edge_pose, sizeof(int32_t) * (size_t)E) && host_block_view(d->edge_point, sizeof(int32_t) * (size_t)E) && host_block_view(d->obs, sizeof(double) * 2 * (size_t)E) && host_block_view(d->inv_sigma2, sizeof(double) * (size_t)E) &&
                     host_block_view(d->poses, sizeof(double) * 7 * (size_t)NP) && host_block_view(d->points, sizeof(double) * 3 * (size_t)P) &&
                     (!d->obs_right || host_block_view(d->obs_right, sizeof(double) * (size_t)E));
    }
    post_helper();
    if (dev_first) {
        rc = group_on_device(); if (rc) return rc;
        ent_packed = s().E_free < kEntPackSlots && P < kEntPackPoints && !HOOK(h, entries_unpacked);
        dev_structure = true;
        rc = after_counts(); if (rc) return rc;
        choose_solver();
        rc = lay_out_rest(); if (rc) return rc;
        pack_pairs();
        rc = send_pairs(); if (rc) return rc;
        device_view();
        h->uploaded = true;
        return MOVBA_OK;
    }
    rc = group(); if (rc || done) return rc;
    rc = pack_derived(); if (rc) return rc;
    rc = send_edge_a(); if (rc) return rc;
    const bool on_device = s().already_grouped && s().nfree > 0 && !HOOK(h, host_structure) && E >= kDeviceStructureMinEdges;
    const bool masks_fit = s().nfree <= 80 && struct_lds_fits(s().nfree, NP);
    ent_packed = s().E_free < kEntPackSlots && P < kEntPackPoints && !HOOK(h, entries_unpacked);
    const bool sorted = on_device && !masks_fit && ent_packed && NP <= kSortedMaxPoses && !HOOK(h, no_sorted_structure);
    dev_structure = on_device && (masks_fit || sorted);
    rc = !dev_structure ? structure_on_host() : (masks_fit ? structure_on_device() : structure_on_device_sorted()); if (rc) return rc;
    if (!edge_b_queued) { rc = queue_edge_b(); if (rc) return rc; }
    choose_solver();
    rc = lay_out_rest(); if (rc) return rc;
    pack_pairs();
    rc = send_pairs(); if (rc) return rc;
    device_view();
    h->uploaded = true;
    return MOVBA_OK;
}

}

extern "C" {

int movba_lba_upload(movba_handle *h, const movba_lba_desc *d)
{
    if (!h || !d) return MOVBA_ERR_ARG;
    int rc;
    {
        Upload u(h, d);
        rc = u.run(true);
    }
    if (rc == kRetryClassic) {
        Upload u(h, d);
        rc = u.run(false);
    }
    if (rc == MOVBA_OK) h->pose_fixed.assign(d->pose_fixed, d->pose_fixed + (d->pose_fixed ? d->n_poses : 0));
    return rc;
}

int movba_lba_reset(movba_handle *h)
{
    if (!h) return MOVBA_ERR_ARG;
    if (!h->uploaded) return MOVBA_ERR_STATE;
    h->ran = false;
    return MOVBA_OK;
}

}
```

Before: 9532 LM iterations/s.

## Streamline host-side structure building with radix sort and direct lane-plan layout

Rewrites the host-side Schur item and schedule construction to drop repeated push_back growth: it pre-sizes vectors, caches per-item weights and wave counts, and replaces per-segment std::sort on 64-bit keys with a byte-wise radix sort on 32-bit keys. The schedule is filled in one pass that also records item slots and destination indices, and coarse-block lists are built by counting sort instead of per-bucket vectors. The PCG lane plan is written directly into the staging buffer, using the recorded item slots rather than a separate rescan of the schedule. The goal is less host time spent on per-window structure setup, at the cost of more intricate bookkeeping and extra temporary buffers whose ordering must match the old logic.

```diff
diff --git a/mov-slam_amd/csrc/kernels.h b/mov-slam_amd/csrc/kernels.h
--- a/mov-slam_amd/csrc/kernels.h
+++ b/mov-slam_amd/csrc/kernels.h
@@ -26,6 +26,8 @@
                               unsigned long long *vals_in, void *tmp, size_t tmp_bytes, long long noff, hipStream_t s);
 hipError_t launch_slot_point(int32_t *slot, const int32_t *g_pose, const int32_t *base, const int32_t *g_point, int32_t *slot_point, int E, const int32_t *hx, int NP, hipStream_t s);
 bool pcg_rows_supported(int nfree, const int32_t *row_ptr, PcgParams *pp);
+constexpr size_t kLanePlanWords = (size_t)kPcgRowsThreads * 12;
+void lay_out_lanes(Structure &s, PcgParams &pp, bool rows_kernel, int32_t *lane_plan);
 hipError_t launch_pcg_rows(const DevWindow &w, int nrowent, const PcgParams &pp, int trial, hipStream_t s);
 
 hipError_t launch_init(const DevWindow &w, hipStream_t s);
diff --git a/mov-slam_amd/csrc/pcg_plan.cpp b/mov-slam_amd/csrc/pcg_plan.cpp
--- a/mov-slam_amd/csrc/pcg_plan.cpp
+++ b/mov-slam_amd/csrc/pcg_plan.cpp
@@ -64,4 +64,38 @@
     return true;
 }
 
+void lay_out_lanes(Structure &s, PcgParams &pp, bool rows_kernel, int32_t *lane_plan)
+{
+    if (!rows_kernel) return;
+    const int nf = s.nfree;
+    const bool on_chip = !pp.overflow;
+    const int32_t *rp = s.row_ptr.data(), *pis = s.pair_item_start.data();
+    const RowEnt *row_ent = s.row_ent.data();
+    for (int wv = 0; wv < kNW; ++wv) {
+        const int r0 = pp.wave_row0[wv], r1 = pp.wave_row0[wv + 1];
+        const int P0 = rp[r0] >> 1, P1 = rp[r1] >> 1;
+        for (int ln = 0; ln < 64; ++ln) {
+            const int t = wv * 64 + ln;
+            int32_t *pl = lane_plan + (size_t)t * 12;
+            for (int k = 0; k < 2; ++k, pl += 4) {
+                const RowEnt *re = P0 + ln < P1 ? &row_ent[2 * (P0 + ln) + k] : nullptr;
+                if (!re || re->block < 0) { pl[0] = pl[1] = pl[2] = pl[3] = -1; continue; }
+                const int32_t i0 = pis[re->block], i1 = pis[re->block + 1];
+                pl[0] = re->block; pl[1] = (re->col * 6) | (re->transposed ? (1 << 30) : 0);
+                pl[2] = i0; pl[3] = i1;
+                if (!on_chip || re->block < nf || i1 - i0 != 1) continue;
+                SchedItem &si = s.sched[(size_t)s.item_slot[(size_t)i0]];
+                const int32_t dst = 36 * k * kPcgRowsThreads + t;
+                if (re->transposed) si.dst_b = dst; else si.dst_a = dst;
+            }
+            pl[0] = pl[1] = pl[2] = pl[3] = 0;
+            if (ln >= 6 * (r1 - r0)) continue;
+            const int bi = r0 + ln / 6;
+            pl[0] = pis[bi]; pl[1] = pis[bi + 1]; pl[2] = rp[bi]; pl[3] = rp[bi + 1];
+        }
+    }
+    for (int wv = 0; wv <= kNW; ++wv) pp.wave_ent0[wv] = rp[pp.wave_row0[wv]];
+    pp.nrowent = rp[nf];
 }
+
+}
diff --git a/mov-slam_amd/csrc/structure.cpp b/mov-slam_amd/csrc/structure.cpp
--- a/mov-slam_amd/csrc/structure.cpp
+++ b/mov-slam_amd/csrc/structure.cpp
@@ -9,7 +9,7 @@
 void reset_structure(Structure& s, int NP, int P, int E)
 {
     s.nfree = 0; s.npairs = 0; s.nitems = 0; s.max_degree = 0; s.nentries = 0; s.already_grouped = true; s.n_fixed = 0; s.n_agg = 0; s.reordered = false;
-    s.free_pose.clear(); s.pair_i.clear(); s.pair_j.clear(); s.items.clear(); s.sched.clear(); s.sched_per_xcd = 0; s.row_ent.clear();
+    s.free_pose.clear(); s.pair_i.clear(); s.pair_j.clear(); s.items.clear(); s.sched_per_xcd = 0; s.rec_slots = 1;
     s.cblk_g.clear(); s.cblk_h.clear(); s.cblk_ptr.clear(); s.cblk_ent.clear(); s.ent_i.clear(); s.ent_j.clear(); s.ent_l.clear(); s.E_free = 0;
     s.NP = NP; s.P = P; s.E = E;
 }
@@ -125,63 +125,32 @@
 int finish_pairs(Structure& s, const int32_t* cnt)
 {
     const int nf = s.nfree;
-    s.pid.assign((size_t)nf * (size_t)nf, -1);
-    s.pair_i.clear(); s.pair_j.clear();
-    for (int i = 0; i < nf; ++i) { s.pid[(size_t)i * nf + i] = i; s.pair_i.push_back(i); s.pair_j.push_back(i); }
-    for (int i = 0; i < nf; ++i)
-        for (int j = i + 1; j < nf; ++j)
-            if (cnt[(size_t)i * nf + j] > 0) {
-                s.pid[(size_t)i * nf + j] = (int32_t)s.pair_i.size();
-                s.pair_i.push_back(i); s.pair_j.push_back(j);
-            }
-    s.npairs = (int)s.pair_i.size();
-    s.pair_ptr.assign(s.npairs + 1, 0);
-    for (int p = 0; p < s.npairs; ++p) s.pair_ptr[p + 1] = s.pair_ptr[p] + cnt[(size_t)s.pair_i[p] * nf + s.pair_j[p]];
+    {
+        const size_t maxp = (size_t)nf + (size_t)nf * (size_t)(nf > 0 ? nf - 1 : 0) / 2;
+        s.pid.resize((size_t)nf * (size_t)nf);
+        s.pair_i.resize(maxp); s.pair_j.resize(maxp); s.pair_ptr.resize(maxp + 1);
+        int32_t *pi = s.pair_i.data(), *pj = s.pair_j.data();
+        int64_t *pp = s.pair_ptr.data();
+        pp[0] = 0;
+        for (int i = 0; i < nf; ++i) { pi[i] = i; pj[i] = i; pp[i + 1] = pp[i] + cnt[(size_t)i * nf + i]; }
+        int np = nf;
+        for (int i = 0; i < nf; ++i) {
+            int32_t *row = s.pid.data() + (size_t)i * nf;
+            const int32_t *crow = cnt + (size_t)i * nf;
+            for (int j = 0; j < i; ++j) row[j] = -1;
+            row[i] = i;
+            for (int j = i + 1; j < nf; ++j) {
+                if (crow[j] > 0) { row[j] = np; pi[np] = i; pj[np] = j; pp[np + 1] = pp[np] + crow[j]; ++np; }
+                else row[j] = -1;
+            }
+        }
+        s.npairs = np;
+        s.pair_i.resize((size_t)np); s.pair_j.resize((size_t)np); s.pair_ptr.resize((size_t)np + 1);
+    }
     s.nentries = s.pair_ptr[s.npairs];
     if (s.nentries > (int64_t)0x7fffffff) return MOVBA_ERR_ARG;
     if (nf > 0 && s.pair_ptr[nf] != (int64_t)s.E_free) return MOVBA_ERR_ARG;
 
-    s.items.clear();
-    s.pair_item_start.assign(s.npairs + 1, 0);
-    for (int p = 0; p < s.npairs; ++p) {
-        const int64_t cap = p < nf ? kSchurChunkDiag : kSchurChunk, len = s.pair_ptr[p + 1] - s.pair_ptr[p];
-        const int64_t parts = (len + cap - 1) / cap;
-        const int64_t chunk = parts > 0 ? ((len + parts - 1) / parts + 3) / 4 * 4 : cap;
-        s.pair_item_start[p] = (int32_t)s.items.size();
-        for (int64_t b = s.pair_ptr[p]; b < s.pair_ptr[p + 1]; b += chunk)
-            s.items.push_back(Item{ p, (int32_t)b, (int32_t)std::min<int64_t>(b + chunk, s.pair_ptr[p + 1]), p < nf ? 1 : 0 });
-    }
-    s.pair_item_start[s.npairs] = (int32_t)s.items.size();
-    s.nitems = (int)s.items.size();
-
-    {
-        const int ipw = kSchurWaves / kSchurWPI;
-        std::vector<int32_t>& order = s.tmp_order;
-        order.resize(s.nitems);
-        {
-            int n = 0, od = nf < s.npairs ? s.pair_item_start[nf] : s.nitems;
-            for (int i = 0; i < nf; ++i) {
-                for (int k = s.pair_item_start[i]; k < s.pair_item_start[i + 1]; ++k) order[n++] = k;
-                while (od < s.nitems && s.pair_i[s.items[od].pair] == i) order[n++] = od++;
-            }
-        }
-        auto weight = [&](int k) { const Item& it = s.items[k]; return (int64_t)(it.end - it.begin) * (it.diag ? 3 : 2) + 128; };
-        int64_t total = 0;
-        for (int k = 0; k < s.nitems; ++k) total += weight(k);
-        std::vector<uint64_t>& key = s.tmp_key;
-        key.resize(s.nitems);
-        int seg_begin[9];
-        {
-            int64_t acc = 0; int x = 0;
-            seg_begin[0] = 0;
-            for (int n = 0; n < s.nitems; ++n) {
-                while (x < 7 && acc >= (total * (x + 1)) / 8) seg_begin[++x] = n;
-                const int64_t wgt = weight(order[n]);
-                key[n] = ((uint64_t)(0x7fffffff - wgt) << 32) | (uint32_t)n;
-                acc += wgt;
-            }
-            while (x < 8) seg_begin[++x] = s.nitems;
-        }
 #ifndef MOVBA_SCHUR_T1
 #define MOVBA_SCHUR_T1 128
 #define MOVBA_SCHUR_T2 256
@@ -189,52 +158,142 @@
 #ifndef MOVBA_SCHUR_DW
 #define MOVBA_SCHUR_DW 4
 #endif
-        auto waves_of = [&](int k) { const Item& it = s.items[k]; const int n = it.end - it.begin; return it.diag ? MOVBA_SCHUR_DW : (n > MOVBA_SCHUR_T2 ? 4 : (n > MOVBA_SCHUR_T1 ? 2 : 1)); };
+    int64_t total = 0;
+    {
+        const size_t bound = (size_t)s.npairs + (size_t)(s.nentries / std::min(kSchurChunkDiag, kSchurChunk)) + 1;
+        s.items.resize(bound); s.tmp_item.resize(2 * bound);
+        s.pair_item_start.resize((size_t)s.npairs + 1);
+        Item *items = s.items.data();
+        int32_t *wn = s.tmp_item.data(), *pis = s.pair_item_start.data();
+        const int64_t *pp = s.pair_ptr.data();
+        int rec = 1, ni = 0;
+        auto add = [&](int p, int64_t b, int64_t e, int diag) {
+            const int n = (int)(e - b);
+            const int32_t wgt = n * (diag ? 3 : 2) + 128;
+            items[ni] = Item{ p, (int32_t)b, (int32_t)e, diag };
+            wn[2 * ni] = wgt;
+            wn[2 * ni + 1] = diag ? MOVBA_SCHUR_DW : (n > MOVBA_SCHUR_T2 ? 4 : (n > MOVBA_SCHUR_T1 ? 2 : 1));
+            total += wgt;
+            ++ni;
+        };
+        for (int p = 0; p < s.npairs; ++p) {
+            const int diag = p < nf ? 1 : 0;
+            const int64_t cap = diag ? kSchurChunkDiag : kSchurChunk, pb = pp[p], pe = pp[p + 1], len = pe - pb;
+            const int first = ni;
+            pis[p] = first;
+            if (len <= cap) { if (len > 0) add(p, pb, pe, diag); }
+            else {
+                const int64_t parts = (len + cap - 1) / cap;
+                const int64_t chunk = ((len + parts - 1) / parts + 3) / 4 * 4;
+                for (int64_t b = pb; b < pe; b += chunk) add(p, b, std::min<int64_t>(b + chunk, pe), diag);
+            }
+            if (diag) rec = std::max(rec, ni - first);
+        }
+        s.items.resize((size_t)ni); s.tmp_item.resize(2 * (size_t)ni);
+        s.pair_item_start[s.npairs] = (int32_t)s.items.size();
+        s.nitems = (int)s.items.size();
+        s.rec_slots = rec;
+    }
+
+    {
+        const int nitems = s.nitems;
+        const Item *items = s.items.data();
+        const int32_t *wn = s.tmp_item.data(), *pis = s.pair_item_start.data();
+        s.tmp_order.resize((size_t)nitems); s.tmp_key.resize((size_t)3 * nitems); s.tmp_pos.resize((size_t)nitems); s.item_slot.resize((size_t)nitems);
+        int32_t *order = s.tmp_order.data(), *pos = s.tmp_pos.data();
+        {
+            int n = 0, od = nf < s.npairs ? pis[nf] : nitems;
+            for (int i = 0; i < nf; ++i) {
+                for (int k = pis[i]; k < pis[i + 1]; ++k) order[n++] = k;
+                while (od < nitems && s.pair_i[items[od].pair] == i) order[n++] = od++;
+            }
+        }
+        constexpr int kMaxWeight = std::max(3 * (kSchurChunkDiag + 3), 2 * (kSchurChunk + 3)) + 128;
+        constexpr uint64_t kKeySpan = 8ull * (kMaxWeight + 1);
+        static_assert(kKeySpan <= 0xffffffffull, "schur item weights beyond a 32-bit sort key");
+        constexpr int kPasses = kKeySpan <= (1ull << 8) ? 1 : kKeySpan <= (1ull << 16) ? 2 : kKeySpan <= (1ull << 24) ? 3 : 4;
+        int seg_begin[9];
+        uint32_t *rkey = s.tmp_key.data();
+        uint32_t *buf[2] = { rkey + nitems, rkey + 2 * (size_t)nitems };
+        {
+            int64_t acc = 0; int x = 0;
+            seg_begin[0] = 0;
+            for (int n = 0; n < nitems; ++n) {
+                while (x < 7 && acc >= (total * (x + 1)) / 8) seg_begin[++x] = n;
+                const int32_t wgt = wn[2 * order[n]];
+                rkey[n] = (uint32_t)x * (uint32_t)(kMaxWeight + 1) + (uint32_t)(kMaxWeight - wgt);
+                buf[0][n] = (uint32_t)n;
+                acc += wgt;
+            }
+            while (x < 8) seg_begin[++x] = nitems;
+        }
+        const uint32_t *sorted = buf[0];
+        for (int pass = 0; pass < kPasses; ++pass) {
+            const int shift = 8 * pass;
+            uint32_t *from = buf[pass & 1], *to = buf[(pass & 1) ^ 1];
+            int32_t start[257] = { 0 };
+            for (int n = 0; n < nitems; ++n) start[((rkey[n] >> shift) & 0xff) + 1]++;
+            for (int v = 0; v < 256; ++v) start[v + 1] += start[v];
+            for (int n = 0; n < nitems; ++n) { const uint32_t q = from[n]; to[start[(rkey[q] >> shift) & 0xff]++] = q; }
+            sorted = to;
+        }
         size_t longest = 1;
-        for (int g = 0; g < 8; ++g) {
-            std::sort(key.begin() + seg_begin[g], key.begin() + seg_begin[g + 1]);
-            size_t slots = 0;
-            for (int n = seg_begin[g]; n < seg_begin[g + 1]; ++n) {
-                const size_t nw = (size_t)waves_of(order[(uint32_t)key[n]]);
-                if ((slots & 3) + nw > 4) slots = (slots + 3) & ~(size_t)3;
-                slots += nw;
-            }
-            longest = std::max(longest, (slots + 3) & ~(size_t)3);
-        }
-        (void)ipw;
-        s.sched_per_xcd = (int)longest;
-        s.sched.assign((size_t)8 * s.sched_per_xcd, SchedItem{ 0, 0, -1, 0, 0, -1, -1, 0 });
         for (int g = 0; g < 8; ++g) {
             size_t slots = 0;
             for (int n = seg_begin[g]; n < seg_begin[g + 1]; ++n) {
-                const int item = order[(uint32_t)key[n]];
-                const Item& it = s.items[item];
-                const int nw = waves_of(item);
-                if ((slots & 3) + (size_t)nw > 4) slots = (slots + 3) & ~(size_t)3;
-                const int len = it.end - it.begin, epw = (len + nw - 1) / nw;
-                for (int sub = 0; sub < nw; ++sub) {
-                    const int wb = std::min(it.begin + sub * epw, it.end), we = std::min(wb + epw, it.end);
-                    s.sched[(size_t)g * s.sched_per_xcd + slots + sub] = SchedItem{ wb, we, (item << 1) | (it.diag ? 1 : 0),
-                                                                                   s.free_pose[s.pair_i[it.pair]], s.free_pose[s.pair_j[it.pair]], -1, -1, sub | (nw << 8) };
+                const size_t nw = (size_t)wn[2 * order[sorted[n]] + 1];
+                if ((slots & 3) + nw > 4) slots = (slots + 3) & ~(size_t)3;
+                pos[n] = (int32_t)slots;
+                slots += nw;
+            }
+            longest = std::max(longest, (slots + 3) & ~(size_t)3);
+        }
+        s.sched_per_xcd = (int)longest;
+        s.sched.resize((size_t)8 * longest);
+        const SchedItem padding{ 0, 0, -1, 0, 0, -1, -1, 0 };
+        const int32_t *fp = s.free_pose.data(), *pi = s.pair_i.data(), *pj = s.pair_j.data();
+        int32_t *item_slot = s.item_slot.data();
+        const int rec_slots = s.rec_slots;
+        for (int g = 0; g < 8; ++g) {
+            SchedItem *seg = s.sched.data() + (size_t)g * longest;
+            size_t filled = 0;
+            for (int n = seg_begin[g]; n < seg_begin[g + 1]; ++n) {
+                const int item = order[sorted[n]];
+                const Item it = items[item];
+                const int nw = wn[2 * item + 1];
+                const size_t at = (size_t)pos[n];
+                while (filled < at) seg[filled++] = padding;
+                const int32_t tag = (item << 1) | (it.diag ? 1 : 0), pose_i = fp[pi[it.pair]], pose_j = fp[pj[it.pair]];
+                const int32_t dst_a = it.diag ? it.pair * rec_slots + (item - pis[it.pair]) : -1;
+                if (nw == 1) seg[at] = SchedItem{ it.begin, it.end, tag, pose_i, pose_j, dst_a, -1, 1 << 8 };
+                else {
+                    const int len = it.end - it.begin, epw = (len + nw - 1) / nw;
+                    for (int sub = 0; sub < nw; ++sub) {
+                        const int wb = std::min(it.begin + sub * epw, it.end), we = std::min(wb + epw, it.end);
+                        seg[at + sub] = SchedItem{ wb, we, tag, pose_i, pose_j, dst_a, -1, sub | (nw << 8) };
+                    }
                 }
-                slots += (size_t)nw;
-            }
+                item_slot[item] = (int32_t)((size_t)g * longest + at);
+                filled = at + (size_t)nw;
+            }
+            while (filled < longest) seg[filled++] = padding;
         }
     }
 
     {
         s.row_ptr.assign(nf + 1, 0);
-        for (int p = 0; p < s.npairs; ++p) {
-            s.row_ptr[s.pair_i[p] + 1]++;
-            if (p >= nf) s.row_ptr[s.pair_j[p] + 1]++;
-        }
-        for (int i = 0; i < nf; ++i) s.row_ptr[i + 1] = s.row_ptr[i] + ((s.row_ptr[i + 1] + 1) & ~1);
-        s.row_ent.assign((size_t)s.row_ptr[nf], RowEnt{ -1, 0, 0, 0 });
-        std::vector<int32_t>& cur = s.tmp_order;
-        cur.assign(s.row_ptr.begin(), s.row_ptr.begin() + nf);
-        for (int p = nf; p < s.npairs; ++p) s.row_ent[cur[s.pair_j[p]]++] = RowEnt{ p, s.pair_i[p], 1, 0 };
-        for (int i = 0; i < nf; ++i) s.row_ent[cur[i]++] = RowEnt{ i, i, 0, 0 };
-        for (int p = nf; p < s.npairs; ++p) s.row_ent[cur[s.pair_i[p]]++] = RowEnt{ p, s.pair_j[p], 0, 0 };
+        int32_t *rp = s.row_ptr.data();
+        const int32_t *pi = s.pair_i.data(), *pj = s.pair_j.data();
+        for (int p = nf; p < s.npairs; ++p) { rp[pi[p] + 1]++; rp[pj[p] + 1]++; }
+        s.tmp_order.resize((size_t)nf);
+        int32_t *cur = s.tmp_order.data();
+        for (int i = 0; i < nf; ++i) { cur[i] = rp[i]; rp[i + 1] = rp[i] + ((rp[i + 1] + 1 + 1) & ~1); }
+        s.row_ent.resize((size_t)rp[nf]);
+        RowEnt *re = s.row_ent.data();
+        for (int p = nf; p < s.npairs; ++p) re[cur[pj[p]]++] = RowEnt{ p, pi[p], 1, 0 };
+        for (int i = 0; i < nf; ++i) re[cur[i]++] = RowEnt{ i, i, 0, 0 };
+        for (int p = nf; p < s.npairs; ++p) re[cur[pi[p]]++] = RowEnt{ p, pj[p], 0, 0 };
+        for (int i = 0; i < nf; ++i) if (cur[i] < rp[i + 1]) re[cur[i]] = RowEnt{ -1, 0, 0, 0 };
     }
     return MOVBA_OK;
 }
@@ -244,50 +303,78 @@
     new_of_old.resize(nf);
     for (int i = 0; i < nf; ++i) new_of_old[i] = i;
     if (nf < 3) return false;
-    auto linked = [&](int a, int b) { return a == b ? false : (a < b ? cnt[(size_t)a * nf + b] : cnt[(size_t)b * nf + a]) > 0; };
-    std::vector<int32_t> deg(nf, 0);
-    for (int i = 0; i < nf; ++i) for (int j = i + 1; j < nf; ++j) if (cnt[(size_t)i * nf + j] > 0) { deg[i]++; deg[j]++; }
-    auto envelope = [&](const std::vector<int32_t>& old_of_new) {
-        int64_t env = 0;
-        for (int r = 0; r < nf; ++r) {
-            int first = r;
-            for (int c = 0; c < r; ++c) if (linked(old_of_new[r], old_of_new[c])) { first = c; break; }
-            env += r - first;
-        }
-        return env;
+    constexpr int kStackNf = 128, kStackW = kStackNf / 64;
+    const int W = (nf + 63) >> 6;
+    uint64_t bits_stack[(size_t)kStackNf * kStackW + 2 * kStackW];
+    int32_t ints_stack[4 * kStackNf];
+    std::vector<uint64_t> bits_heap;
+    std::vector<int32_t> ints_heap;
+    uint64_t *bits = bits_stack;
+    int32_t *ints = ints_stack;
+    if (nf > kStackNf) {
+        bits_heap.resize((size_t)nf * W + 2 * (size_t)W); ints_heap.resize(4 * (size_t)nf);
+        bits = bits_heap.data(); ints = ints_heap.data();
+    }
+    uint64_t *adj = bits, *placed = bits + (size_t)nf * W, *seen = placed + W;
+    int32_t *deg = ints, *level = ints + nf, *queue = ints + 2 * (size_t)nf, *order = ints + 3 * (size_t)nf;
+    std::memset(adj, 0, sizeof(uint64_t) * ((size_t)nf * W + W));
+    for (int i = 0; i < nf; ++i) {
+        const int32_t *crow = cnt + (size_t)i * nf;
+        for (int j = i + 1; j < nf; ++j)
+            if (crow[j] > 0) { adj[(size_t)i * W + (j >> 6)] |= 1ull << (j & 63); adj[(size_t)j * W + (i >> 6)] |= 1ull << (i & 63); }
+    }
+    for (int i = 0; i < nf; ++i) {
+        int dg = 0;
+        for (int w = 0; w < W; ++w) dg += __builtin_popcountll(adj[(size_t)i * W + w]);
+        deg[i] = dg;
+    }
+    int nq = 0;
+    auto bfs = [&](int root) {
+        for (int w = 0; w < W; ++w) seen[w] = placed[w];
+        seen[root >> 6] |= 1ull << (root & 63);
+        queue[0] = root; nq = 1; level[root] = 0;
+        for (int h = 0; h < nq; ++h) {
+            const int v = queue[h], first = nq;
+            for (int w = 0; w < W; ++w) {
+                uint64_t f = adj[(size_t)v * W + w] & ~seen[w];
+                seen[w] |= f;
+                for (; f; f &= f - 1) { const int u = (w << 6) + __builtin_ctzll(f); level[u] = level[v] + 1; queue[nq++] = u; }
+            }
+            if (nq - first > 1) std::sort(queue + first, queue + nq, [&](int a, int b) { return deg[a] != deg[b] ? deg[a] < deg[b] : a < b; });
+        }
+        return level[queue[nq - 1]];
     };
-    std::vector<int32_t> order, level(nf), queue;
-    std::vector<uint8_t> placed(nf, 0);
-    auto bfs = [&](int root, std::vector<int32_t>& out) {
-        out.clear(); out.push_back(root);
-        std::fill(level.begin(), level.end(), -1); level[root] = 0;
-        for (size_t h = 0; h < out.size(); ++h) {
-            const int v = out[h];
-            const size_t first = out.size();
-            for (int u = 0; u < nf; ++u) if (!placed[u] && level[u] < 0 && linked(v, u)) { level[u] = level[v] + 1; out.push_back(u); }
-            std::sort(out.begin() + first, out.end(), [&](int a, int b) { return deg[a] != deg[b] ? deg[a] < deg[b] : a < b; });
-        }
-        return level[out.back()];
-    };
-    order.reserve(nf);
+    int n_order = 0;
     for (;;) {
         int root = -1;
-        for (int i = 0; i < nf; ++i) if (!placed[i] && (root < 0 || deg[i] < deg[root])) root = i;
+        for (int i = 0; i < nf; ++i) if (!((placed[i >> 6] >> (i & 63)) & 1) && (root < 0 || deg[i] < deg[root])) root = i;
         if (root < 0) break;
         for (int sweep = 0; sweep < 2; ++sweep) {
-            const int depth = bfs(root, queue);
+            const int depth = bfs(root);
             int far = -1;
-            for (int v : queue) if (level[v] == depth && (far < 0 || deg[v] < deg[far])) far = v;
+            for (int q = 0; q < nq; ++q) { const int v = queue[q]; if (level[v] == depth && (far < 0 || deg[v] < deg[far])) far = v; }
             if (far == root) break;
             root = far;
         }
-        bfs(root, queue);
-        for (int v : queue) { placed[v] = 1; order.push_back(v); }
-    }
-    std::reverse(order.begin(), order.end());
-    std::vector<int32_t> natural(nf);
-    for (int i = 0; i < nf; ++i) natural[i] = i;
-    const int64_t env_nat = envelope(natural), env_rcm = envelope(order);
+        bfs(root);
+        for (int q = 0; q < nq; ++q) { const int v = queue[q]; placed[v >> 6] |= 1ull << (v & 63); order[n_order++] = v; }
+    }
+    std::reverse(order, order + nf);
+    int64_t env_nat = 0, env_rcm = 0;
+    for (int r = 0; r < nf; ++r)
+        for (int w = 0; w <= (r >> 6); ++w) {
+            const uint64_t f = adj[(size_t)r * W + w];
+            if (f) { const int c = (w << 6) + __builtin_ctzll(f); if (c < r) env_nat += r - c; break; }
+        }
+    int32_t *at = level;
+    for (int k = 0; k < nf; ++k) at[order[k]] = k;
+    for (int r = 0; r < nf; ++r) {
+        const int v = order[r];
+        int first = r;
+        for (int w = 0; w < W; ++w)
+            for (uint64_t f = adj[(size_t)v * W + w]; f; f &= f - 1) first = std::min(first, (int)at[(w << 6) + __builtin_ctzll(f)]);
+        env_rcm += r - first;
+    }
     if (!(env_rcm * 5 < env_nat * 4)) return false;
     for (int k = 0; k < nf; ++k) new_of_old[order[k]] = k;
     return true;
@@ -296,14 +383,16 @@
 void apply_pose_order(Structure& s, const std::vector<int32_t>& new_of_old, int32_t* cnt)
 {
     const int nf = s.nfree;
-    std::vector<int32_t> fp(nf);
+    std::vector<int32_t>& fp = s.tmp_order;
+    fp.resize(nf);
     for (int h = 0; h < nf; ++h) fp[new_of_old[h]] = s.free_pose[h];
-    s.free_pose = fp;
+    std::copy(fp.begin(), fp.end(), s.free_pose.begin());
     for (int h = 0; h < nf; ++h) s.hidx[s.free_pose[h]] = h;
     int run = 0;
     for (int h = 0; h < nf; ++h) { s.pose_slot0[s.free_pose[h]] = run; run += s.pose_edges[s.free_pose[h]]; }
     if (cnt) {
-        std::vector<int32_t> c2((size_t)nf * nf, 0);
+        std::vector<int32_t>& c2 = s.tmp_cnt;
+        c2.assign((size_t)nf * nf, 0);
         for (int i = 0; i < nf; ++i)
             for (int j = i; j < nf; ++j) {
                 const int a = new_of_old[i], b = new_of_old[j];
@@ -329,7 +418,7 @@
             for (int b = a; b < fe_start[l + 1]; ++b) row[fe_h[b]]++;
         }
     if (nf <= 80 && !s.no_reorder) {
-        std::vector<int32_t> new_of_old;
+        std::vector<int32_t>& new_of_old = s.tmp_perm;
         if (covisibility_order(nf, cnt.data(), new_of_old)) {
             apply_pose_order(s, new_of_old, nullptr);
             build_slots(s);
@@ -369,33 +458,40 @@
 {
     const int nf = s.nfree, G = n_agg;
     s.n_agg = G;
-    s.cblk_g.clear(); s.cblk_h.clear(); s.cblk_ent.clear(); s.cblk_ij.clear(); s.cblk_ptr.assign(1, 0);
     s.multi_pairs.clear();
+    const int32_t *pis = s.pair_item_start.data();
     for (int p = nf; p < s.npairs; ++p)
-        if (s.pair_item_start[p + 1] - s.pair_item_start[p] > 1) s.multi_pairs.push_back(p);
-    std::vector<int32_t> agg_of(nf, 0);
+        if (pis[p + 1] - pis[p] > 1) s.multi_pairs.push_back(p);
+    s.tmp_order.resize((size_t)nf); s.tmp_pos.assign((size_t)G * G + 1, 0);
+    int32_t *agg_of = s.tmp_order.data(), *start = s.tmp_pos.data();
+    for (int i = 0; i < nf; ++i) agg_of[i] = 0;
     for (int g = 0; g < G; ++g)
         for (int i = agg_row0[g]; i < agg_row0[g + 1]; ++i) agg_of[i] = g;
-    std::vector<std::vector<int32_t>> lists((size_t)G * G), ijs((size_t)G * G);
+    const RowEnt *re = s.row_ent.data();
+    const int32_t *rp = s.row_ptr.data();
     for (int i = 0; i < nf; ++i)
-        for (int e = s.row_ptr[i]; e < s.row_ptr[i + 1]; ++e)
-            if (s.row_ent[e].block >= 0) {
-                const size_t b = (size_t)agg_of[i] * G + agg_of[s.row_ent[e].col];
-                const int pr = s.row_ent[e].block;
-                const bool single = pr >= nf && s.pair_item_start[pr + 1] - s.pair_item_start[pr] == 1;
-                const int src_idx = single ? s.pair_item_start[pr] : pr;
-                lists[b].push_back((src_idx << 2) | (s.row_ent[e].transposed ? 2 : 0) | (single ? 1 : 0));
-                ijs[b].push_back((i << 16) | s.row_ent[e].col);
-            }
+        for (int e = rp[i]; e < rp[i + 1]; ++e)
+            if (re[e].block >= 0) start[(size_t)agg_of[i] * G + agg_of[re[e].col] + 1]++;
+    s.cblk_g.clear(); s.cblk_h.clear(); s.cblk_ptr.assign(1, 0);
     for (int g = 0; g < G; ++g)
         for (int h = 0; h < G; ++h) {
-            const std::vector<int32_t>& l = lists[(size_t)g * G + h];
-            if (l.empty()) continue;
-            s.cblk_g.push_back(g); s.cblk_h.push_back(h);
-            s.cblk_ent.insert(s.cblk_ent.end(), l.begin(), l.end());
-            s.cblk_ij.insert(s.cblk_ij.end(), ijs[(size_t)g * G + h].begin(), ijs[(size_t)g * G + h].end());
-            s.cblk_ptr.push_back((int32_t)s.cblk_ent.size());
-        }
-}
-
-}
+            const size_t b = (size_t)g * G + h;
+            const int32_t n = start[b + 1];
+            start[b + 1] = start[b] + n;
+            if (n == 0) continue;
+            s.cblk_g.push_back(g); s.cblk_h.push_back(h); s.cblk_ptr.push_back(start[b + 1]);
+        }
+    s.cblk_ent.resize((size_t)start[(size_t)G * G]); s.cblk_ij.resize((size_t)start[(size_t)G * G]);
+    for (int i = 0; i < nf; ++i)
+        for (int e = rp[i]; e < rp[i + 1]; ++e)
+            if (re[e].block >= 0) {
+                const int32_t at = start[(size_t)agg_of[i] * G + agg_of[re[e].col]]++;
+                const int pr = re[e].block;
+                const bool single = pr >= nf && pis[pr + 1] - pis[pr] == 1;
+                const int src_idx = single ? pis[pr] : pr;
+                s.cblk_ent[at] = (src_idx << 2) | (re[e].transposed ? 2 : 0) | (single ? 1 : 0);
+                s.cblk_ij[at] = (i << 16) | re[e].col;
+            }
+}
+
+}
diff --git a/mov-slam_amd/csrc/structure.h b/mov-slam_amd/csrc/structure.h
--- a/mov-slam_amd/csrc/structure.h
+++ b/mov-slam_amd/csrc/structure.h
@@ -27,7 +27,9 @@
     std::vector<int32_t> hidx;
     std::vector<int32_t> free_pose;
     std::vector<int32_t> perm;
-    std::vector<int32_t> tmp_order; std::vector<uint64_t> tmp_key;
+    std::vector<int32_t> tmp_order; std::vector<uint32_t> tmp_key;
+    std::vector<int32_t> tmp_item, tmp_pos;
+    std::vector<int32_t> tmp_perm, tmp_cnt;
     std::vector<int32_t> pose_edges, pose_slot0;
     std::vector<int32_t> pt_start;
     std::vector<int32_t> g_pose, g_point;
@@ -40,6 +42,8 @@
     std::vector<int32_t> ent_i, ent_j, ent_l;
     int E_free = 0;
     std::vector<Item> items;
+    std::vector<int32_t> item_slot;
+    int rec_slots = 1;
     std::vector<SchedItem> sched;
     int sched_per_xcd = 0;
     std::vector<int32_t> row_ptr;
diff --git a/mov-slam_amd/csrc/upload.cpp b/mov-slam_amd/csrc/upload.cpp
--- a/mov-slam_amd/csrc/upload.cpp
+++ b/mov-slam_amd/csrc/upload.cpp
@@ -126,7 +126,7 @@
     size_t o_obspm = 0, o_obsrpm = 0, o_part = 0, o_blocks = 0, o_blocks_ov = 0, o_blocks_c = 0, o_aci = 0, o_acitag = 0;
     size_t o_bp = 0, o_xp = 0, o_scale = 0, o_hmax = 0, o_tick = 0, o_recd = 0, o_imgb = 0, o_ctrl = 0, o_chi2 = 0, o_outl = 0;
     size_t o_dtiles = 0, o_ddiag = 0, o_dfail = 0, o_dx = 0, o_dflags = 0, o_dcontrib = 0, o_dstamps = 0;
-    std::vector<int32_t> lane_plan;
+    size_t plan_words = 0;
     int rec_slots = 1;
     size_t ncb = 0;
     int ntile = 0;
@@ -585,7 +585,7 @@
     if (cnt[nbins] != 0) return MOVBA_ERR_ARG;
     lap("wait for the pair counts");
     if (!h->st.no_reorder) {
-        std::vector<int32_t> new_of_old;
+        std::vector<int32_t> &new_of_old = h->st.tmp_perm;
         if (covisibility_order(nf, cnt, new_of_old)) {
             apply_pose_order(h->st, new_of_old, cnt);
             h->st.reordered = true;
@@ -764,52 +764,10 @@
     o_items = c.take<Item>((size_t)s().nitems + 1); o_sched = c.take<SchedItem>(s().sched.size() + 1);
     o_pi = c.take<int32_t>(s().npairs + 1); o_pj = c.take<int32_t>(s().npairs + 1); o_pis = c.take<int32_t>(s().npairs + 1);
     o_rowptr = c.take<int32_t>(nf + 1); o_rowent = c.take<RowEnt>(s().row_ent.size() + 1);
-    lane_plan.clear();
-    if (h->rows_kernel) {
-        lane_plan.assign((size_t)kPcgRowsThreads * 12, -1);
-        for (int wv = 0; wv < kPcgRowsThreads / 64; ++wv) {
-            const int r0 = h->pp.wave_row0[wv], r1 = h->pp.wave_row0[wv + 1];
-            const int P0 = s().row_ptr[r0] >> 1, P1 = s().row_ptr[r1] >> 1;
-            for (int ln = 0; ln < 64 && P0 + ln < P1; ++ln)
-                for (int k = 0; k < 2; ++k) {
-                    const RowEnt &re = s().row_ent[2 * (P0 + ln) + k];
-                    int32_t *pl = &lane_plan[((size_t)(wv * 64 + ln) * 3 + k) * 4];
-                    if (re.block < 0) continue;
-                    pl[0] = re.block; pl[1] = (re.col * 6) | (re.transposed ? (1 << 30) : 0);
-                    pl[2] = s().pair_item_start[re.block]; pl[3] = s().pair_item_start[re.block + 1];
-                }
-            for (int ln = 0; ln < 64; ++ln) {
-                int32_t *pl = &lane_plan[((size_t)(wv * 64 + ln) * 3 + 2) * 4];
-                pl[0] = pl[1] = pl[2] = pl[3] = 0;
-                if (ln >= 6 * (r1 - r0)) continue;
-                const int bi = r0 + ln / 6;
-                pl[0] = s().pair_item_start[bi]; pl[1] = s().pair_item_start[bi + 1]; pl[2] = s().row_ptr[bi]; pl[3] = s().row_ptr[bi + 1];
-            }
-        }
-        for (int wv = 0; wv <= kPcgRowsThreads / 64; ++wv) h->pp.wave_ent0[wv] = s().row_ptr[h->pp.wave_row0[wv]];
-        h->pp.nrowent = s().row_ptr[nf];
-    }
-    rec_slots = 1;
-    for (int hh = 0; hh < nf; ++hh) rec_slots = std::max(rec_slots, (int)(s().pair_item_start[hh + 1] - s().pair_item_start[hh]));
-    for (SchedItem &si : h->st.sched) {
-        si.dst_a = -1; si.dst_b = -1;
-        if (si.tag >= 0 && (si.tag & 1)) { const Item &it = s().items[(size_t)(si.tag >> 1)]; si.dst_a = it.pair * rec_slots + ((si.tag >> 1) - s().pair_item_start[it.pair]); }
-    }
-    if (h->rows_kernel && !h->pp.overflow) {
-        std::vector<int32_t> slot_of_item((size_t)s().nitems, -1);
-        for (size_t q = 0; q < s().sched.size(); ++q)
-            if (s().sched[q].tag >= 0 && (s().sched[q].sub & 0xff) == 0) slot_of_item[(size_t)(s().sched[q].tag >> 1)] = (int32_t)q;
-        for (int t = 0; t < kPcgRowsThreads; ++t)
-            for (int k = 0; k < 2; ++k) {
-                const int32_t *pl = &lane_plan[((size_t)t * 3 + k) * 4];
-                if (pl[0] < nf || pl[3] - pl[2] != 1) continue;
-                SchedItem &si = h->st.sched[(size_t)slot_of_item[(size_t)pl[2]]];
-                const int32_t dst = 36 * k * kPcgRowsThreads + t;
-                if ((pl[1] >> 30) & 1) si.dst_b = dst; else si.dst_a = dst;
-            }
-    }
+    plan_words = h->rows_kernel ? kLanePlanWords : 0;
+    rec_slots = s().rec_slots;
     ncb = s().cblk_g.size();
-    o_plan = c.take<int32_t>(lane_plan.size() + 4);
+    o_plan = c.take<int32_t>(plan_words + 4);
     o_cg = c.take<int32_t>(ncb + 1); o_ch = c.take<int32_t>(ncb + 1); o_cp = c.take<int32_t>(ncb + 2); o_ce = c.take<int32_t>(s().cblk_ent.size() + 1);
     o_cij = c.take<int32_t>(s().cblk_ij.size() + 1); o_multi = c.take<int32_t>(s().multi_pairs.size() + 1);
     o_pid = c.take<int32_t>((size_t)nf * nf + 1);
@@ -863,6 +821,7 @@
             put(eh + 2 * noff, s().ent_l.data(), sizeof(int32_t) * noff);
         }
     }
+    lay_out_lanes(h->st, h->pp, h->rows_kernel, reinterpret_cast<int32_t *>(sp(o_plan)));
     put(sp(o_items), s().items.data(), sizeof(Item) * (size_t)s().nitems);
     put(sp(o_sched), s().sched.data(), sizeof(SchedItem) * s().sched.size());
     put(sp(o_pi), s().pair_i.data(), sizeof(int32_t) * s().npairs);
@@ -870,7 +829,6 @@
     put(sp(o_pis), s().pair_item_start.data(), sizeof(int32_t) * (s().npairs + 1));
     put(sp(o_rowptr), s().row_ptr.data(), sizeof(int32_t) * (nf + 1));
     put(sp(o_rowent), s().row_ent.data(), sizeof(RowEnt) * s().row_ent.size());
-    if (!lane_plan.empty()) put(sp(o_plan), lane_plan.data(), sizeof(int32_t) * lane_plan.size());
     put(sp(o_cg), s().cblk_g.data(), sizeof(int32_t) * ncb);
     put(sp(o_ch), s().cblk_h.data(), sizeof(int32_t) * ncb);
     put(sp(o_cp), s().cblk_ptr.data(), sizeof(int32_t) * s().cblk_ptr.size());
```

Result: slower. 9291 LM iterations/s (-2.5%).
